# ecmwf-ifs/ectrans

Hardware: AMD Instinct MI355X
Metric: dir+inv transform-pairs/sec, TCo1279 137L x 10 fields; spectral-norm rel-error (higher is better)
Workload: dtype f64

## Files before the change

### ectrans_amd/__init__.py

```python
import ctypes as C
import os

import numpy as np

__all__ = ["TransError", "setup_trans0", "setup_trans", "inv_trans", "dir_trans", "trans_inq", "specnorm",
           "trans_release", "trans_end", "lib", "build", "esetup_trans", "einv_trans", "edir_trans", "etrans_inq"]

_HERE = os.path.dirname(os.path.abspath(__file__))
_LIBPATH = os.path.join(_HERE, "libectrans_mi.so")
_L = None

EMI_MEM_HOST, EMI_MEM_DEVICE, EMI_MEM_AUTO = 0, 1, 2


class TransError(RuntimeError):
    """What the reference would have reported through ABORT_TRANS."""


class _Init(C.Structure):
    _fields_ = [("kmax_resol", C.c_int), ("kprintlev", C.c_int), ("prad", C.c_double), ("nproc", C.c_int),
                ("myproc", C.c_int), ("device", C.c_int), ("nprtrv", C.c_int)]


class _VSets(C.Structure):
    _fields_ = [("kvsetuv", C.POINTER(C.c_int)), ("nuv_g", C.c_int), ("kvsetsc", C.POINTER(C.c_int)), ("nsc_g", C.c_int),
                ("kvsetsc2", C.POINTER(C.c_int)), ("nsc2_g", C.c_int), ("kvsetsc3a", C.POINTER(C.c_int)), ("nsc3a_g", C.c_int),
                ("kvsetsc3b", C.POINTER(C.c_int)), ("nsc3b_g", C.c_int), ("nvar3a_g", C.c_int), ("nvar3b_g", C.c_int)]


class _LegpolIO(C.Structure):
    _fields_ = [("io", C.c_char_p), ("fname", C.c_char_p), ("ptr", C.c_void_p), ("len", C.c_size_t)]


class _Setup(C.Structure):
    _fields_ = [("ksmax", C.c_int), ("kdgl", C.c_int), ("kloen", C.POINTER(C.c_int)), ("kdlon", C.c_int),
                ("precision", C.c_int), ("lduseflt", C.c_int), ("ldll", C.c_int), ("ldstretch", C.c_int),
                ("lduserpnm", C.c_int), ("ldshiftll", C.c_int)]


class _ESetup(C.Structure):
    _fields_ = [("kmsmax", C.c_int), ("ksmax", C.c_int), ("kdgl", C.c_int), ("kloen", C.POINTER(C.c_int)), ("kdlon", C.c_int),
                ("kdgux", C.c_int), ("pexwn", C.c_double), ("peywn", C.c_double), ("precision", C.c_int)]


class _Ext(C.Structure):
    _fields_ = [("sp_dim2", C.c_int), ("gp", C.c_int * 3), ("gpuv", C.c_int * 4), ("gp3a", C.c_int * 4),
                ("gp3b", C.c_int * 4), ("gp2", C.c_int * 3)]


class _Inv(C.Structure):
    _fields_ = [("mem_space", C.c_int), ("spvor", C.c_void_p), ("spdiv", C.c_void_p), ("nf_uv", C.c_int),
                ("spscalar", C.c_void_p), ("nf_scalar", C.c_int), ("spsc3a", C.c_void_p), ("sc3a_nlev", C.c_int),
                ("sc3a_nvar", C.c_int), ("spsc3b", C.c_void_p), ("sc3b_nlev", C.c_int), ("sc3b_nvar", C.c_int),
                ("spsc2", C.c_void_p), ("nf_sc2", C.c_int), ("ldscders", C.c_int), ("ldvorgp", C.c_int),
                ("lddivgp", C.c_int), ("lduvder", C.c_int), ("kproma", C.c_int), ("gp", C.c_void_p),
                ("gp_nfld", C.c_int), ("gpuv", C.c_void_p), ("gp3a", C.c_void_p), ("gp3b", C.c_void_p),
                ("gp2", C.c_void_p), ("stream", C.c_void_p), ("ext", C.POINTER(_Ext)), ("vsets", C.POINTER(_VSets)),
                ("ldlatlon", C.c_int)]


class _Dir(C.Structure):
    _fields_ = [("mem_space", C.c_int), ("spvor", C.c_void_p), ("spdiv", C.c_void_p), ("nf_uv", C.c_int),
                ("spscalar", C.c_void_p), ("nf_scalar", C.c_int), ("spsc3a", C.c_void_p), ("sc3a_nlev", C.c_int),
                ("sc3a_nvar", C.c_int), ("spsc3b", C.c_void_p), ("sc3b_nlev", C.c_int), ("sc3b_nvar", C.c_int),
                ("spsc2", C.c_void_p), ("nf_sc2", C.c_int), ("kproma", C.c_int), ("gp", C.c_void_p),
                ("gp_nfld", C.c_int), ("gpuv", C.c_void_p), ("gp3a", C.c_void_p), ("gp3b", C.c_void_p),
                ("gp2", C.c_void_p), ("stream", C.c_void_p), ("ext", C.POINTER(_Ext)), ("vsets", C.POINTER(_VSets))]


def build(force=False):
    import subprocess
    src = os.path.join(_HERE, "csrc", "ectrans_mi.hip")
    deps = [src] + [os.path.join(_HERE, "csrc", f) for f in ("emi_kernels.h", "emi_kernels_body.h", "emi_mr_body.h", "emi_mr_tables.h", "emi_types.h", "emi_rt.h", "emi_setup.h", "emi_stage.h")]
    deps.append(os.path.join(os.path.dirname(_HERE), "include", "ectrans_mi.h"))
    if not force and os.path.exists(_LIBPATH) and all(os.path.getmtime(_LIBPATH) >= os.path.getmtime(d) for d in deps):
        return _LIBPATH
    hipcc = os.environ.get("HIPCC", "/opt/rocm/bin/hipcc")
    cmd = [hipcc, "--offload-arch=gfx950", "-O3", "-std=c++17", "-fPIC", "-shared", "-o", _LIBPATH, src]
    subprocess.check_call(cmd)
    return _LIBPATH


def source_hash():
    import hashlib
    h = hashlib.sha256()
    files = sorted(os.path.join(_HERE, "csrc", f) for f in os.listdir(os.path.join(_HERE, "csrc")))
    files.append(os.path.join(os.path.dirname(_HERE), "include", "ectrans_mi.h"))
    for f in files:
        if os.path.isfile(f):
            h.update(os.path.basename(f).encode() + b"\0" + open(f, "rb").read())
    return h.hexdigest()[:16]


def _bind(L):
    ip, dp = C.POINTER(C.c_int), C.POINTER(C.c_double)
    L.emi_init.argtypes = [C.POINTER(_Init)]
    L.emi_setup.argtypes = [C.POINTER(_Setup), ip]
    L.emi_setup_legpol.argtypes = [C.POINTER(_Setup), C.POINTER(_LegpolIO), ip]
    L.emi_inq_int.argtypes = [C.c_int, C.c_char_p, ip]
    L.emi_inq_int_array.argtypes = [C.c_int, C.c_char_p, ip, C.c_int]
    L.emi_inq_real_array.argtypes = [C.c_int, C.c_char_p, dp, C.c_int]
    L.emi_inq_legendre.argtypes = [C.c_int, C.c_int, C.c_int, dp, ip, ip]
    L.emi_inv_trans.argtypes = [C.c_int, C.POINTER(_Inv)]
    L.emi_dir_trans.argtypes = [C.c_int, C.POINTER(_Dir)]
    L.emi_specnorm.argtypes = [C.c_int, C.c_int, C.c_void_p, C.c_int, dp]
    L.emi_inv_transad.argtypes = [C.c_int, C.POINTER(_Inv)]
    L.emi_dir_transad.argtypes = [C.c_int, C.POINTER(_Dir)]
    L.emi_release.argtypes = [C.c_int]
    L.emi_finalize.argtypes = []
    L.emi_trim_cache.argtypes = []
    L.emi_last_error.restype = C.c_char_p
    L.emi_work_model.argtypes = [C.c_int, C.c_int, dp, dp, dp]
    L.emi_last_phase_ms.argtypes = [dp]
    L.emi_set_max_batch.argtypes = [C.c_int]
    L.emi_specnorm_partial.argtypes = [C.c_int, C.c_int, C.c_void_p, C.c_int, dp]
    L.emi_gpnorm.argtypes = [C.c_int, C.c_int, C.c_void_p, C.c_int, C.c_int, C.c_int, dp, dp, dp, C.c_int]
    L.emi_vordiv_to_uv.argtypes = [C.c_int, C.c_int, C.c_int, C.c_void_p, C.c_void_p, C.c_void_p, C.c_void_p, C.c_int, C.c_int]
    if hasattr(L, "emi_ptr_space"):
        L.emi_ptr_space.argtypes = [C.c_void_p]
        L.emi_wait.argtypes = [C.c_int]
    L.emi_specnorm_kvset.argtypes = [C.c_int, C.c_int, C.c_void_p, C.c_int, C.POINTER(C.c_int), C.c_int, dp]
    L.emi_set_alltoallv.argtypes = [C.c_void_p, C.c_void_p]
    L.emi_set_profile.argtypes = [C.c_int]
    L.emi_last_phase_launches.argtypes = [ip]
    if hasattr(L, "emi_last_exchange"):
        L.emi_last_exchange.argtypes = [dp, ip, dp]
        L.emi_last_fft_launches.argtypes = [C.POINTER(C.c_longlong)]
    L.emi_crc64.argtypes = [C.c_void_p, C.c_size_t, C.POINTER(C.c_ulonglong)]
    L.emi_set_host_collectives.argtypes = [C.c_void_p, C.c_void_p, C.c_void_p]
    L.emi_dist_spec.argtypes = [C.c_int, C.c_void_p, C.c_int, ip, ip, C.c_void_p]
    L.emi_gath_spec.argtypes = [C.c_int, C.c_void_p, C.c_int, ip, C.c_void_p]
    L.emi_dist_grid.argtypes = [C.c_int, C.c_void_p, C.c_int, ip, ip, C.c_int, C.c_void_p]
    L.emi_gath_grid.argtypes = [C.c_int, C.c_void_p, C.c_int, ip, C.c_int, C.c_void_p]
    L.emi_inq_tasks.argtypes = [ip, ip]
    L.emi_inq_init.argtypes = [ip, dp]
    L.emi_set_nprtrv.argtypes = [C.c_int]
    if hasattr(L, "emi_esetup"):
        L.emi_esetup.argtypes = [C.POINTER(_ESetup), ip]
        L.emi_einv_trans.argtypes = [C.c_int, C.POINTER(_Inv), C.c_void_p, C.c_void_p]
        L.emi_edir_trans.argtypes = [C.c_int, C.POINTER(_Dir), C.c_void_p, C.c_void_p]
    return L


def lib():
    global _L
    if _L is None:
        if not os.path.exists(_LIBPATH):
            raise TransError("libectrans_mi.so is not built (run __graft_entry__.build()); "
                             "ectrans_amd has no CPU implementation")
        _L = _bind(C.CDLL(_LIBPATH))
    return _L


def _use_library_for_tests(path):
    global _L
    _L = _bind(C.CDLL(path))
    return _L


def _chk(rc):
    if rc != 0:
        raise TransError(lib().emi_last_error().decode())


def _is_torch(a):
    return a is not None and type(a).__module__.startswith("torch")


def _ptr(a, space):
    if a is None:
        return None, None
    if _is_torch(a):
        if not a.is_contiguous() or str(a.dtype) != "torch." + space[1]:
            raise TransError("device arrays must be contiguous %s tensors" % space[1])
        if space[0] is None:
            space[0] = EMI_MEM_DEVICE if a.is_cuda else EMI_MEM_HOST
        elif space[0] != (EMI_MEM_DEVICE if a.is_cuda else EMI_MEM_HOST):
            raise TransError("all arrays of one call must live in the same memory space")
        return a.data_ptr(), a
    if not (isinstance(a, np.ndarray) and a.dtype == np.dtype(space[1]) and a.flags.c_contiguous):
        raise TransError("host arrays must be C-contiguous %s numpy arrays" % space[1])
    if space[0] is None:
        space[0] = EMI_MEM_HOST
    elif space[0] != EMI_MEM_HOST:
        raise TransError("all arrays of one call must live in the same memory space")
    return a.ctypes.data, a


def _space(mem_space, space):
    return int(mem_space) if mem_space is not None else space[0] if space[0] is not None else EMI_MEM_HOST


_DIST = {"nproc": 1, "nprtrv": 1, "group": None, "device": None}


def setup_trans0(kmax_resol=1, kprintlev=0, prad=None, device=-1, kprtrw=1, myproc=1, group=None, alltoallv=None,
                 transport="torch", kprtrv=1, **unsupported):
    for k, v in unsupported.items():
        if k.lower() in ("kprgpns", "kprgpew") and v not in (None, 1, kprtrw, kprtrw * kprtrv):
            raise TransError("SETUP_TRANS0: %s=%r: only the W-set decomposition (KPRTRW tasks) is supported" % (k, v))
    nproc_all = kprtrw * max(1, kprtrv)
    if transport == "rccl":
        from . import dist as _dist
        if kprtrv > 1:
            _chk(lib().emi_set_nprtrv(int(kprtrv)))
        _dist.rccl_native_attach(nproc_all, myproc, kmax_resol, kprintlev, prad, device, group)
        _DIST.update(nproc=nproc_all, nprtrv=max(1, kprtrv), group=group if nproc_all > 1 else None,
                     device=("cuda:%d" % device) if nproc_all > 1 and device is not None and device >= 0 else None)
        return
    if nproc_all > 1:
# ... 439 lines not shown
    dt = real_dtype(kresol)
    ns2g, me = trans_inq(kresol, "nspec2g"), trans_inq(kresol, "myproc")
    kto = _roots(kto, kfgathg, "GATH_SPEC:KTO")
    loc = np.ascontiguousarray(_np(pspec), dtype=dt)
    nm = int((kto == me).sum())
    g = np.zeros((nm, ns2g), dtype=dt) if nm else None
    _chk(lib().emi_gath_spec(kresol, None if g is None else g.ctypes.data, kfgathg, _iptr(kto), loc.ctypes.data))
    return None if g is None else np.ascontiguousarray(g.T)


def gath_grid(kresol, pgp, kfgathg, kto=1):
    dt = real_dtype(kresol)
    ngg, me = trans_inq(kresol, "ngptotg"), trans_inq(kresol, "myproc")
    kto = _roots(kto, kfgathg, "GATH_GRID:KTO")
    loc = np.ascontiguousarray(_np(pgp), dtype=dt)
    if loc.ndim != 3 or loc.shape[1] != kfgathg:
        raise TransError("GATH_GRID: PGP must have shape (ngpblks, kfgathg=%d, nproma)" % kfgathg)
    nm = int((kto == me).sum())
    g = np.zeros((nm, ngg), dtype=dt) if nm else None
    _chk(lib().emi_gath_grid(kresol, None if g is None else g.ctypes.data, kfgathg, _iptr(kto), loc.shape[2], loc.ctypes.data))
    return g


def dist_grid(kresol, pgpg, kfdistg, kfrom=1, kproma=None):
    dt = real_dtype(kresol)
    ngl, ngg, me = trans_inq(kresol, "ngptot"), trans_inq(kresol, "ngptotg"), trans_inq(kresol, "myproc")
    kfrom = _roots(kfrom, kfdistg, "DIST_GRID:KFROM")
    mine = np.flatnonzero(kfrom == me)
    g = None
    if mine.size:
        a = _np(pgpg)
        if a.shape[-1] != ngg:
            raise TransError("DIST_GRID: PGPG must have shape (nfld, ngptotg=%d)" % ngg)
        g = np.ascontiguousarray(a[mine], dtype=dt)
    nproma = int(kproma) if kproma else ngl
    out = np.zeros(((ngl - 1) // nproma + 1, kfdistg, nproma), dtype=dt)
    _chk(lib().emi_dist_grid(kresol, None if g is None else g.ctypes.data, kfdistg, _iptr(kfrom), None, nproma, out.ctypes.data))
    return out


def trans_release(kresol):
    _chk(lib().emi_release(kresol))


def trim_cache():
    _chk(lib().emi_trim_cache())


def trans_end():
    _chk(lib().emi_finalize())
    _DIST.update(nproc=1, nprtrv=1, group=None, device=None)


def work_model(kresol, nfields):
    a, b, c = C.c_double(), C.c_double(), C.c_double()
    _chk(lib().emi_work_model(kresol, nfields, C.byref(a), C.byref(b), C.byref(c)))
    return {"legendre_flops": a.value, "fft_flops": b.value, "fourier_bytes": c.value}


def last_phase_ms():
    out = (C.c_double * 3)()
    lib().emi_last_phase_ms(out)
    return list(out)


def last_phase_launches():
    out = (C.c_int * 3)()
    lib().emi_last_phase_launches(out)
    return list(out)


def last_exchange():
    ms, n, b = C.c_double(), C.c_int(), C.c_double()
    lib().emi_last_exchange(C.byref(ms), C.byref(n), C.byref(b))
    return ms.value, n.value, b.value


def last_fft_launches():
    k = C.c_longlong()
    lib().emi_last_fft_launches(C.byref(k))
    return k.value


def set_profile(on):
    lib().emi_set_profile(int(on))


def set_max_batch(n):
    lib().emi_set_max_batch(int(n))
```

### ectrans_amd/csrc/ectrans_mi.hip

```cpp
#include <atomic>
#include <chrono>
#include <cmath>
#include <cstdarg>
#include <cstdio>
#include <map>
#include <memory>
#include <string>
#include <vector>

#include <fcntl.h>
#include <sys/mman.h>
#include <sys/stat.h>
#include <unistd.h>

#include "../../include/ectrans_mi.h"
#include "emi_kernels.h"
#include "emi_setup.h"
#include <dlfcn.h>

struct EmiRoctx {
  int (*push)(const char *) = nullptr;
  int (*pop)() = nullptr;
  bool tried = false;
  void load() {
// ... 131 lines not shown
#ifdef EMI_CPU_EMU
  (void)p;
  return EMI_MEM_HOST;
#else
  if (!p) return EMI_MEM_HOST;
  hipPointerAttribute_t at;
  if (hipPointerGetAttributes(&at, p) != hipSuccess) {
    (void)hipGetLastError();
    return EMI_MEM_HOST;
  }
  return (at.type == hipMemoryTypeDevice || at.type == hipMemoryTypeManaged || at.type == hipMemoryTypeArray) ? EMI_MEM_DEVICE : EMI_MEM_HOST;
#endif
}
static int agree_on_mixed_arrays(const char *who, int ndev, int nhost);
static int resolve_space(const char *who, int mem_space, std::initializer_list<const void *> arrays, int *out, bool collective = false) {
  if (mem_space == EMI_MEM_HOST || mem_space == EMI_MEM_DEVICE) {
    *out = mem_space;
    return 0;
  }
  if (mem_space != EMI_MEM_AUTO) EMI_FAIL(EMI_ERR_ARG, "%s: mem_space = %d (EMI_MEM_HOST, EMI_MEM_DEVICE or EMI_MEM_AUTO)", who, mem_space);
  int ndev = 0, nhost = 0;
  for (const void *q : arrays)
    if (q) (emi_ptr_space(q) == EMI_MEM_DEVICE ? ndev : nhost)++;
  if (collective) {
    if (agree_on_mixed_arrays(who, ndev, nhost)) return EMI_ERR_ARG;
  } else if (ndev && nhost) {
    EMI_FAIL(EMI_ERR_ARG, "%s: %d ARRAYS OF THE CALL ARE IN DEVICE MEMORY AND %d IN HOST MEMORY (all of them must live in one place)", who, ndev, nhost);
  }
  *out = ndev ? EMI_MEM_DEVICE : EMI_MEM_HOST;
  return 0;
}

template <class T>
static int upload(const std::vector<T> &h, T **d) {
  void *p = nullptr;
  if (emi_dev_malloc(&p, h.size() * sizeof(T))) return -1;
  if ((!h.empty() && emi_h2d(p, h.data(), h.size() * sizeof(T), 0)) || emi_stream_sync(0)) {
    emi_dev_free(p);
    return -1;
  }
  *d = (T *)p;
  return 0;
}
struct DevAllocs {
  std::vector<void *> list;
  DevAllocs() = default;
  DevAllocs(const DevAllocs &) = delete;
  DevAllocs &operator=(const DevAllocs &) = delete;
  ~DevAllocs() {
    for (void *p : list) emi_dev_free(p);
  }
  int alloc(void **p, size_t bytes) {
    if (emi_dev_malloc(p, bytes)) return -1;
    list.push_back(*p);
    return 0;
  }
};
template <class T, class F>
static int upload(DevAllocs &owner, const std::vector<T> &h, F *field) {
  T *d = nullptr;
  if (upload(h, &d)) return -1;
  owner.list.push_back(d);
  *field = d;
  return 0;
}

#define EMI_LAUNCH_P(esz, kern, grid, block, lds, st, ...)                     \
  do {                                                                         \
    if ((esz) == 8) {                                                          \
      typedef double RT;                                                       \
      EMI_LAUNCH(emi_f64::kern, grid, block, lds, st, __VA_ARGS__);            \
    } else {                                                                   \
      typedef float RT;                                                        \
      EMI_LAUNCH(emi_f32::kern, grid, block, lds, st, __VA_ARGS__);            \
    }                                                                          \
  } while (0)

struct FftClass {
  int nthr = 0, fbk = 0;
  int hot = 0;
  int r16 = 0;
  int split = 0;
  int mr = 0;
  int gmem = 0;
  long long gm_elems = 0;
  std::vector<int> lats;
  int *d_lats = nullptr;
  FftRowDev *d_rows = nullptr;
  size_t lds = 0;
};
struct LegMaps {
  int2 *d_inv = nullptr, *d_dir = nullptr, *d_inv_wide = nullptr, *d_dir_wide = nullptr;
  long long n_inv = 0, n_dir = 0, n_inv_wide = 0, n_dir_wide = 0;
};

struct Plan {
  Plan() = default;
  Plan(const Plan &) = delete;
  Plan &operator=(const Plan &) = delete;
  ~Plan();
  int nsmax = 0, ndgl = 0, ndgnh = 0;
  bool reduced = false;
  bool ldll = false, shiftll = false;
  bool lam = false;
  int lam_n = 0, kdgux = 0;
  double exwn = 0.0, eywn = 0.0;
  std::vector<int> kntmp;
  std::vector<int> l_kntmp, nesm0;
  LamDev lamdev{};
  int lam_nthr = 0;
  size_t lam_lds = 0;
  double ra = 6371229.0;
  std::vector<int> nloen, nmen, ndglu, procm;
  std::vector<int> latlo;
  std::vector<double> rmu, rw, racthe, cos2;
  int ngptotg = 0, nspec2g = 0;
  int nproc = 1, me = 0;
  int nprv = 1, mev = 0;
  std::vector<int> vlat;
  int vfirst(int w, int v) const { return nprv > 1 ? vlat[(size_t)w * nprv + v] : latlo[w]; }
  int vlast(int w, int v) const { return nprv > 1 ? vlat[(size_t)w * nprv + v + 1] : latlo[w + 1]; }
  long long vpoints(int w, int v) const {
    long long c = 0;
    for (int j = vfirst(w, v); j < vlast(w, v); j++) c += nloen[j];
    return c;
  }
  long long voffset(int v) const {
    long long c = 0;
    for (int j = latlo[me]; j < vfirst(me, v); j++) c += nloen[j];
    return c;
  }
  int nump = 0, nlat = 0, lat0 = 0;
  int ngptot = 0, nspec2 = 0;
  std::vector<int> mval, nasm0;
  std::vector<int> l_nmen, l_gpoff, l_fbase;
  std::vector<int> wbase, wrows, ldp, ldk, lattile_pref, ktile_pref, lbase;
  std::vector<long long> offS, offA, offTS, offTA;
  long long frows = 0, lrows = 0, wrows_total = 0, p_elems = 0, pt_elems = 0;
  std::vector<long long> leg_rows, leg_disp, fft_rows, fft_disp;
  EmiGeomDev g{};
  DevAllocs dev_allocs;
  int esz = 8;
  char *d_P = nullptr, *d_PT = nullptr;
  std::vector<FftPlanDev> fplans;
  std::vector<int> planid;
  FftTabDev ftab{};
  std::vector<FftClass> fclass;
  std::map<int, LegMaps> legmaps;
  char *d_W = nullptr, *d_FBL = nullptr, *d_FBF = nullptr;
  size_t cap_W = 0, cap_FBL = 0, cap_FBF = 0;
  void *d_desc = nullptr;
  size_t cap_desc = 0;
  char *d_fftscr = nullptr;
  size_t cap_fftscr = 0;
#ifndef EMI_CPU_EMU
  hipEvent_t ev_done = nullptr;
#endif
  bool ev_valid = false;
};

Plan::~Plan() {
#ifndef EMI_CPU_EMU
  if (ev_done) (void)hipEventDestroy(ev_done);
#endif
  emi_dev_free(d_W);
  emi_dev_free(d_FBL);
// ... 88 lines not shown
  G.nprtrv = c.nprtrv > 0 ? c.nprtrv : (G.nprtrv_preset > 0 ? G.nprtrv_preset : 1);
  if (G.nproc_all % G.nprtrv != 0)
    EMI_FAIL(EMI_ERR_ARG, "SUMP_TRANS0: NPROC INCONSISTENT WITH NPRTRW (NPROC = %d is not a multiple of NPRTRV = %d)", G.nproc_all, G.nprtrv);
  G.nproc = G.nproc_all / G.nprtrv;
  G.myproc = (G.myproc_all - 1) / G.nprtrv + 1;
  G.mysetv = (G.myproc_all - 1) % G.nprtrv + 1;
#ifndef EMI_CPU_EMU
  int ndev = 0;
  if (hipGetDeviceCount(&ndev) != hipSuccess || ndev == 0)
    EMI_FAIL(EMI_ERR_RUNTIME, "emi_init: no HIP device visible -- libectrans_mi has no CPU path");
  if (c.device >= 0) EMI_CHECK(hipSetDevice(c.device));
#endif
  G.plans.clear();
  G.plans.resize(G.max_resol);
  const char *pe = getenv("EMI_PROFILE");
  G.profile = pe ? atoi(pe) : 0;
  const char *mb = getenv("EMI_MAX_BATCH");
  if (mb) G.max_batch = atoi(mb);
  G.init = true;
  return EMI_SUCCESS;
}


static double mr_radix_ops(int R) {
  switch (R) {
    case 2: return 4; case 3: return 14; case 4: return 16; case 5: return 36; case 7: return 66; case 11: return 150;
    case 13: return 204; case 17: return 336; case 19: return 414; case 23: return 594;
    case 6: return 3 * 4 + 2 * 14 + 12; case 8: return 4 * 4 + 2 * 16 + 18; case 9: return 6 * 14 + 24; case 10: return 5 * 4 + 2 * 36 + 24;
    case 12: return 4 * 14 + 3 * 16 + 36; case 14: return 7 * 4 + 2 * 66 + 36; case 15: return 5 * 14 + 3 * 36 + 48; case 16: return 8 * 16 + 54;
    case 18: return 9 * 4 + 2 * 108 + 48; case 20: return 5 * 16 + 4 * 36 + 72; case 21: return 7 * 14 + 3 * 66 + 72;
    default: return -1;
  }
}
static bool mr_choose(int sz, int esz, int fac[3], int &fbk, int &nthr) {
  std::vector<int> rs = {
#define EMI_MR_ROW(r_) r_,
      EMI_MR_RADICES(EMI_MR_ROW)
  };
#ifdef EMI_MR_RADICES_F32
  if (esz == 4)
    for (int r : {EMI_MR_RADICES_F32(EMI_MR_ROW)}) rs.push_back(r);
#endif
#undef EMI_MR_ROW
  double best = 1e300;
  bool found = false;
  auto consider = [&](int A, int B, int C) {
    const int P1 = (B * C) | 1;
    const size_t per_field = (size_t)A * P1 * 2 * esz;
    if (per_field > 160 * 1024 || A * P1 > 65535) return;
    int fb = 16;
    while (fb > 1 && fb * per_field > 40960) fb >>= 1;
    const int R[3] = {A, B, C};
    for (int nt = 128; nt <= 256; nt += 64) {
      double cost = 0;
      for (int ip = 0; ip < 3; ip++) {
        if (R[ip] == 1) continue;
        const long long nb = (long long)fb * (sz / R[ip]);
        const long long sweeps = (nb + nt - 1) / nt;
        cost += (double)(sweeps * nt) / (double)nb * (mr_radix_ops(R[ip]) / R[ip] + 15.0);
      }
      cost *= 1.0 + 0.5 * (256 - nt) / 64.0;
      if (cost < best * (1.0 - 1e-9) || (cost <= best * (1.0 + 1e-9) && nt > nthr)) {
        best = cost, found = true;
        fac[0] = A, fac[1] = B, fac[2] = C, fbk = fb, nthr = nt;
      }
    }
  };
  for (int A : rs) {
    if (sz % A) continue;
    const int m1 = sz / A;
    if (m1 == 1) consider(A, 1, 1);
    for (int B : rs) {
      if (m1 % B) continue;
      const int C = m1 / B;
      if (C == 1) consider(A, B, 1);
      for (int Cc : rs)
        if (Cc == C) consider(A, B, C);
    }
  }
  return found;
}

struct FftSwitches {
  bool mr, r16, r16s, hot;
  static bool off(const char *name) { return getenv(name) && atoi(getenv(name)) == 0; }
  FftSwitches() : mr(!off("EMI_FFT_MR")), r16(!off("EMI_FFT_R16")), r16s(!off("EMI_FFT_R16S")), hot(!getenv("EMI_FFT_NO_HOT")) {}
};
struct HotPlan {
  int pc, S, nfac, fac[5], nfl;
};
static const HotPlan g_hot_plans[] = {
#define EMI_HOT_ROW(pc_, S_, nf_, a_, b_, c_, d_, e_, nfl_) {pc_, S_, nf_, {a_, b_, c_, d_, e_}, nfl_},
    EMI_HOT_PLAN_LIST(EMI_HOT_ROW)
#undef EMI_HOT_ROW
};
#define EMI_LIST_ROW(r_) r_,
static const int g_r16_list[] = {EMI_R16_LIST(EMI_LIST_ROW)}, g_r16s_list[] = {EMI_R16S_LIST(EMI_LIST_ROW)};
#undef EMI_LIST_ROW

static int fft_fields_40k(size_t per_field) {
  int fbk = 16;
  while (fbk > 1 && fbk * per_field > 40960) fbk >>= 1;
  return fbk;
}
static int fft_threads(size_t lds_bytes) { return lds_bytes <= 40960 ? 256 : (lds_bytes <= 81920 ? 512 : 1024); }

struct FftChoice {
  FftPlanDev pl{};
  int nthr = 0;
  int hot = 0;
  bool gmem = false;
};
static int fft_choose(int n, int esz, const FftSwitches &sw, FftChoice &c) {
  FftPlanDev &pl = c.pl;
  pl.n = n;
  pl.cmode = (n % 2 != 0);
  pl.sz = pl.cmode ? n : n / 2;
  std::vector<int> fac;
  pl.blue = !emi::factorize_smooth(pl.sz, fac);
  pl.S = pl.sz;
  int mr_fbk = 0, mr_nthr = 0, mr_fac[3] = {1, 1, 1};
  if (!pl.cmode && pl.sz >= 2 && sw.mr) pl.mr = mr_choose(pl.sz, esz, mr_fac, mr_fbk, mr_nthr) ? 1 : 0;
  if (pl.mr) {
    pl.blue = 0;
    fac.assign(mr_fac, mr_fac + 3);
  }
  if (!pl.mr && !pl.cmode && sw.r16) {
    const int need = 2 * pl.sz - 1;
    if (need > 1536)
      for (int r : g_r16_list)
        if (!pl.r16 && 256 * r >= need) pl.r16 = r;
    if (!pl.r16 && need > 4096 && pl.sz % 2 == 0 && sw.r16s)
      for (int r : g_r16s_list)
        if (!pl.r16 && 256 * r >= pl.sz - 1) pl.r16 = r, pl.split = 2;
    if (pl.r16) pl.blue = 1;
  }
  if (pl.r16) {
    pl.S = 256 * pl.r16;
    fac.assign(1, pl.r16);
  } else if (pl.blue) {
    pl.S = emi::next_235(2 * pl.sz - 1);
    emi::factorize_smooth(pl.S, fac);
    if (!pl.cmode && sw.hot) {
      long long best = (long long)pl.S * (long long)(fac.size() + 1);
      const HotPlan *pick = nullptr;
      for (const HotPlan &r : g_hot_plans) {
        if (r.S < 2 * pl.sz - 1) continue;
        if (fft_fields_40k((size_t)FFT_LDS_ELEMS(r.S) * 2 * esz) < r.nfl) continue;
        const long long cost = (long long)r.S * (r.nfac + 1);
        if (cost <= best) {
          best = cost;
          pick = &r;
        }
      }
      if (pick) {
        pl.S = pick->S;
        fac.assign(pick->fac, pick->fac + pick->nfac);
      }
    }
  }
  if (pl.S > 65535 || fac.size() > 14) EMI_FAIL(EMI_ERR_UNSUPPORTED, "FFT length %d not supported (work size %d)", n, pl.S);
  pl.nfac = (int)fac.size();
  for (int i = 0; i < pl.nfac; i++) pl.fac[i] = fac[i];
  const size_t per_field = (size_t)FFT_LDS_ELEMS(pl.S) * 2 * esz;
  pl.fbk = fft_fields_40k(per_field);
  c.gmem = pl.fbk * per_field > 160 * 1024 && !pl.mr;
  c.nthr = fft_threads(pl.fbk * per_field);
  if (pl.r16) {
    pl.fbk = 1;
    c.nthr = 16 * pl.r16 > 256 ? roundup(16 * pl.r16, 64) : 256;
  } else if (pl.mr) {
    pl.fbk = mr_fbk;
    c.nthr = mr_nthr;
  } else if (pl.blue && !pl.cmode && !c.gmem && sw.hot) {
    int hot_fbk = 0;
    for (const HotPlan &r : g_hot_plans)
      if (r.S == pl.S && r.nfac == pl.nfac && r.nfl <= pl.fbk && std::equal(r.fac, r.fac + r.nfac, pl.fac)) c.hot = r.pc, hot_fbk = r.nfl;
    if (c.hot) {
      pl.fbk = hot_fbk;
      c.nthr = fft_threads(pl.fbk * per_field);
    }
  }
  for (int i = 0; i < pl.nfac; i++)
    if (!c.hot && !pl.r16 && !pl.mr && (pl.fac[i] == 6 || pl.fac[i] > 8)) EMI_FAIL(EMI_ERR_RUNTIME, "internal: composite FFT radix %d without a specialised kernel (length %d)", pl.fac[i], n);
  return 0;
}

struct FftShared {
  int S, tw_off, perm_off, ptw_off[14];
  std::vector<int> fac;
  int r16 = 0, mr = 0;
};
struct FftTabSizes { size_t tw = 0, ptw = 0, perm = 0, rtw = 0, chirp = 0, bhat = 0; };

static void fft_fill_shared(const FftShared &sh, std::vector<d2> &tw, std::vector<d2> &ptw, std::vector<uint16_t> &perm) {
  const int S = sh.S;
  if (sh.mr) {
    const int A = sh.fac[0], B = sh.fac[1], C = sh.fac[2], P1 = (B * C) | 1;
    auto w = [&](long long e) {
      long double a = 2.0L * (long double)M_PIl * (long double)(e % S) / (long double)S;
      return d2{(double)cosl(a), (double)-sinl(a)};
    };
    d2 *t1 = ptw.data() + sh.ptw_off[0], *t2 = ptw.data() + sh.ptw_off[1];
    for (int k1 = 0; k1 < A; k1++) t1[k1] = w((long long)C * k1);
    for (int q = 0; q < A * B; q++) t2[q] = w((long long)q);
    for (int k = 0; k < S; k++) perm[sh.perm_off + k] = (uint16_t)((k % A) * P1 + ((k / A) % B) * C + k / (A * B));
    return;
  }
  if (sh.r16) {
    d2 *dst = ptw.data() + sh.ptw_off[0];
    for (int row = 0; row < 7; row++) {
      const int mult = row < 3 ? row + 1 : 4 * (row - 2);
      for (int t = 0; t < 256; t++) {
        long double a = 2.0L * (long double)M_PIl * (long double)(((long long)t * mult) % S) / (long double)S;
        *dst++ = d2{(double)cosl(a), (double)-sinl(a)};
      }
    }
    return;
  }
  for (int k = 0; k < S; k++) {
    long double a = 2.0L * (long double)M_PIl * (long double)k / (long double)S;
    tw[sh.tw_off + k] = d2{(double)cosl(a), (double)-sinl(a)};
  }
  long long lenp = 1;
  for (size_t ip = 0; ip < sh.fac.size(); ip++) {
    const int R = sh.fac[ip];
    d2 *dst = ptw.data() + sh.ptw_off[ip];
    if (lenp > 1)
      for (int t = 1; t < R; t++)
        for (long long j = 0; j < lenp; j++) {
          long double a = 2.0L * (long double)M_PIl * (long double)((j * t) % (lenp * R)) / (long double)(lenp * R);
          *dst++ = d2{(double)cosl(a), (double)-sinl(a)};
        }
    lenp *= R;
  }
  std::vector<uint16_t> pm;
  emi::dit_positions(S, sh.fac, pm);
  std::copy(pm.begin(), pm.end(), perm.begin() + sh.perm_off);
}

static void fft_fill_length(const FftPlanDev &pl, const std::vector<uint16_t> &perm, std::vector<d2> &rtw, std::vector<d2> &chirp, std::vector<d2> &bhat) {
  const int n = pl.n;
  const double tpi = 2.0 * M_PI;
  for (int k = 0; k <= pl.sz; k++) {
    double a = tpi * (double)k / (double)n;
    rtw[pl.rtw_off + k] = d2{std::cos(a), -std::sin(a)};
  }
  if (!pl.blue) return;
  d2 *c = chirp.data() + pl.chirp_off;
  const int csz = pl.split ? pl.sz / 2 : pl.sz;
  for (int k = 0; k < csz; k++) {
    long long k2 = ((long long)k * k) % (2LL * csz);
    double a = M_PI * (double)k2 / (double)csz;
    c[k] = d2{std::cos(a), -std::sin(a)};
  }
  const int L = pl.S, r0 = pl.fac[0];
// ... 11 lines not shown
      sr += (long double)c[jj].x * cs;
      si += -(long double)c[jj].y * cs;
    }
    if (pl.r16) {
      const int k0 = k % pl.r16, kk = k / pl.r16, k1 = kk % 16, k2 = kk / 16;
      bh[(size_t)k2 * (16 * pl.r16) + 16 * k0 + k1] = d2{(double)(sr / (long double)L), (double)(si / (long double)L)};
      continue;
    }
    const int p = pm[k];
    bh[(size_t)(p % r0) * (L / r0) + p / r0] = d2{(double)sr, (double)si};
  }
}

static const FftShared &fft_share_tables(const FftPlanDev &pl, std::map<int, int> &sidx, std::vector<FftShared> &shared, FftTabSizes &n) {
  const int skey = pl.S * 16 + (pl.r16 ? 15 : (pl.mr ? 14 : pl.nfac));
  auto si = sidx.find(skey);
  if (si != sidx.end()) return shared[si->second];
  FftShared sh{};
  sh.S = pl.S;
  sh.fac.assign(pl.fac, pl.fac + pl.nfac);
  sh.r16 = pl.r16;
  sh.mr = pl.mr;
  sh.tw_off = (int)n.tw;
  sh.perm_off = (int)n.perm;
  if (pl.mr) {
    const int A = pl.fac[0], B = pl.fac[1];
    sh.ptw_off[0] = (int)n.ptw;
    n.ptw += (size_t)A;
    sh.ptw_off[1] = (int)n.ptw;
    n.ptw += (size_t)A * B;
    sh.ptw_off[2] = (int)n.ptw;
    n.perm += pl.S;
  } else if (pl.r16) {
    sh.ptw_off[0] = (int)n.ptw;
    n.ptw += 7 * 256;
  } else {
    n.tw += pl.S;
    n.perm += pl.S;
    long long lenp = 1;
    for (int ip = 0; ip < pl.nfac; ip++) {
      sh.ptw_off[ip] = (int)n.ptw;
      if (lenp > 1) n.ptw += (size_t)(pl.fac[ip] - 1) * lenp;
      lenp *= pl.fac[ip];
    }
  }
  sidx.emplace(skey, (int)shared.size());
  shared.push_back(sh);
  return shared.back();
}

static int build_fft_plans(Plan &P) {
  const FftSwitches sw;
  std::map<int, int> idx;
  std::map<int, int> sidx;
  std::vector<FftShared> shared;
  FftTabSizes nt;
  P.planid.assign(P.nlat, 0);
  for (int j = 0; j < P.nlat; j++) {
    const int n = P.nloen[P.lat0 + j];
    auto it = idx.find(n);
    if (it != idx.end()) {
      P.planid[j] = it->second;
      continue;
    }
    FftChoice c;
    if (int rc = fft_choose(n, P.esz, sw, c)) return rc;
    FftPlanDev &pl = c.pl;
    const FftShared &sh = fft_share_tables(pl, sidx, shared, nt);
    pl.tw_off = sh.tw_off;
    pl.perm_off = sh.perm_off;
    for (int ip = 0; ip < pl.nfac; ip++) pl.ptw_off[ip] = sh.ptw_off[ip];
    pl.rtw_off = (int)nt.rtw;
    nt.rtw += pl.sz + 1;
    if (pl.blue) {
      pl.chirp_off = (int)nt.chirp;
      nt.chirp += pl.split ? pl.sz / 2 : pl.sz;
      pl.bhat_off = (int)nt.bhat;
      nt.bhat += pl.S;
    }
    if (nt.tw > 0x7fffffffULL || nt.ptw > 0x7fffffffULL || nt.bhat > 0x7fffffffULL) EMI_FAIL(EMI_ERR_UNSUPPORTED, "FFT tables too large");
    int cls = -1;
    for (size_t k = 0; k < P.fclass.size(); k++) {
      const FftClass &fc = P.fclass[k];
      if (fc.nthr == c.nthr && fc.fbk == pl.fbk && fc.hot == c.hot && fc.r16 == pl.r16 && fc.split == pl.split && fc.mr == pl.mr && fc.gmem == (int)c.gmem) cls = (int)k;
    }
    if (cls < 0) {
      cls = (int)P.fclass.size();
      P.fclass.emplace_back();
      FftClass &fc = P.fclass[cls];
      fc.nthr = c.nthr, fc.fbk = pl.fbk, fc.hot = c.hot, fc.r16 = pl.r16, fc.split = pl.split, fc.mr = pl.mr, fc.gmem = c.gmem;
    }
    pl.lds_class = cls;
    idx[n] = P.planid[j] = (int)P.fplans.size();
    P.fplans.push_back(pl);
  }
  if (P.lam) {
    FftPlanDev pl{};
    pl.n = pl.sz = pl.S = P.ndgl;
    pl.cmode = 1;
    std::vector<int> fac;
    pl.blue = !emi::factorize_smooth(pl.sz, fac);
    if (pl.blue) {
      pl.S = emi::next_235(2 * pl.sz - 1);
      emi::factorize_smooth(pl.S, fac);
    }
    const int fs = FFT_LDS_ELEMS(pl.S) + 1, fs_max = 160 * 1024 / (4 * P.esz);
    if (fs > fs_max || pl.S > 65535 || fac.size() > 14)
      EMI_FAIL(EMI_ERR_UNSUPPORTED,
               "ESETUP_TRANS: KDGL = %d NEEDS A WORK ARRAY OF %d COMPLEX NUMBERS PER FIELD (KDGL WHERE IT FACTORISES IN 2, 3, 5, 7, ELSE THE CONVOLUTION LENGTH ABOVE 2 KDGL); THE "
               "Y-DIRECTION KERNELS HOLD TWO FIELDS IN THE 160 KIB OF LDS: AT MOST %d",
               P.ndgl, fs, fs_max);
    pl.nfac = (int)fac.size();
    for (int i = 0; i < pl.nfac; i++) pl.fac[i] = fac[i];
    const size_t per_field = (size_t)fs * 2 * P.esz;
    pl.fbk = std::max(2, std::min(16, (int)(80 * 1024 / per_field) / 2 * 2));
    const FftShared &sh = fft_share_tables(pl, sidx, shared, nt);
    pl.tw_off = sh.tw_off;
    pl.perm_off = sh.perm_off;
    for (int ip = 0; ip < pl.nfac; ip++) pl.ptw_off[ip] = sh.ptw_off[ip];
    pl.rtw_off = (int)nt.rtw;
    nt.rtw += pl.sz + 1;
    if (pl.blue) {
      pl.chirp_off = (int)nt.chirp;
      nt.chirp += pl.sz;
      pl.bhat_off = (int)nt.bhat;
      nt.bhat += pl.S;
    }
    pl.lds_class = -1;
    P.lamdev.yplan = (int)P.fplans.size();
    P.lamdev.fbk = pl.fbk;
    P.lamdev.fs = fs;
    P.lam_lds = (size_t)pl.fbk * per_field;
    P.lam_nthr = std::min(512, fft_threads(P.lam_lds));
    P.fplans.push_back(pl);
  }
  std::vector<d2> tw(nt.tw), rtw(nt.rtw), chirp(nt.chirp), bhat(nt.bhat), ptw(nt.ptw);
  std::vector<uint16_t> perm(nt.perm);
  emi::parallel_for((int)shared.size(), [&](int is) { fft_fill_shared(shared[is], tw, ptw, perm); });
  std::vector<int> order(P.fplans.size());
  for (size_t i = 0; i < order.size(); i++) order[i] = (int)i;
  std::sort(order.begin(), order.end(), [&](int a, int b) { return P.fplans[a].n > P.fplans[b].n; });
  emi::parallel_for((int)order.size(), [&](int io) { fft_fill_length(P.fplans[order[io]], perm, rtw, chirp, bhat); });
  for (int j = 0; j < P.nlat; j++) {
    const FftPlanDev &pl = P.fplans[P.planid[j]];
    FftClass &fc = P.fclass[pl.lds_class];
    fc.lats.push_back(j);
    if (fc.gmem)
      fc.gm_elems = std::max(fc.gm_elems, (long long)pl.fbk * FFT_LDS_ELEMS(pl.S));
    else if (fc.mr)
      fc.lds = std::max(fc.lds, (size_t)pl.fbk * pl.fac[0] * ((pl.fac[1] * pl.fac[2]) | 1) * 2 * P.esz);
    else if (fc.r16)
      fc.lds = (size_t)fc.r16 * 272 * 8 + (size_t)((fc.split ? 128 * fc.r16 : 0) + 240) * 2 * P.esz;
    else
      fc.lds = std::max(fc.lds, (size_t)pl.fbk * FFT_LDS_ELEMS(pl.S) * 2 * P.esz);
  }
  std::vector<d2> tw256(15 * 16);
  for (int k1 = 1; k1 < 16; k1++)
    for (int c = 0; c < 16; c++) {
      long double a = 2.0L * (long double)M_PIl * (long double)(c * k1) / 256.0L;
      tw256[(k1 - 1) * 16 + c] = d2{(double)cosl(a), (double)-sinl(a)};
    }
  auto upload_c = [&](const std::vector<d2> &v, const void **d) {
    if (P.esz == 8) return upload(P.dev_allocs, v, d);
    std::vector<f2> w(v.size());
    for (size_t i = 0; i < v.size(); i++) w[i] = f2{(float)v[i].x, (float)v[i].y};
    return upload(P.dev_allocs, w, d);
  };
  FftTabDev &ft = P.ftab;
  if (upload_c(tw, &ft.tw) || upload_c(ptw, &ft.ptw) || upload_c(rtw, &ft.rtw) || upload_c(chirp, &ft.chirp) || upload_c(bhat, &ft.bhat) || upload_c(tw256, &ft.tw256) ||
      upload(P.dev_allocs, perm, &ft.perm) || upload(P.dev_allocs, P.fplans, &ft.plans) || upload(P.dev_allocs, P.planid, &ft.planid))
    return EMI_ERR_RUNTIME;
  for (FftClass &fc : P.fclass) {
    if (upload(P.dev_allocs, fc.lats, &fc.d_lats)) return EMI_ERR_RUNTIME;
// ... 968 lines not shown
        return EMI_ERR_RUNTIME;
      }
      ok = fwrite(buf.data(), 8, buf.size(), f) == buf.size();
    }
  ok = (fclose(f) == 0) && ok;
  if (!ok) EMI_FAIL(EMI_ERR_RUNTIME, "WRITE_LEGPOL:BYTES_IO_WRITE FAILED (%s)", fname);
  return EMI_SUCCESS;
}

struct HostStage {
  size_t esz;
  explicit HostStage(int e) : esz((size_t)e) {}
  std::vector<void *> dev;
  bool failed = false;
  std::vector<std::pair<void *, std::pair<void *, size_t>>> outs;
  ~HostStage() {
    for (void *p : dev) emi_stage::release(p);
  }
  const void *in(const void *h, size_t elems, bool host, emi_stream_t s) {
    if (!h || !host) return h;
    void *d = emi_stage::acquire(elems * esz);
    if (!d) {
      failed = true;
      return nullptr;
    }
    dev.push_back(d);
    if (emi_h2d(d, h, elems * esz, s)) failed = true;
    return d;
  }
  void *out(void *h, size_t elems, bool host, bool preload = false, emi_stream_t s = 0) {
    if (!h || !host) return h;
    void *d = emi_stage::acquire(elems * esz);
    if (!d) {
      failed = true;
      return nullptr;
    }
    dev.push_back(d);
    if (preload && emi_h2d(d, h, elems * esz, s)) failed = true;
    outs.push_back({d, {h, elems * esz}});
    return d;
  }
  void flush(emi_stream_t s) {
    for (auto &o : outs) emi_d2h(o.second.first, o.first, o.second.second, s);
    emi_stream_sync(s);
  }
};

static int grow(Plan &P, char **p, size_t *cap, size_t need, const char *what, emi_stream_t st) {
  if (need <= *cap) return 0;
  plan_quiesce(P);
  emi_stream_sync(0);
  emi_dev_free(*p);
  *p = nullptr;
  *cap = 0;
  void *q;
  if (emi_dev_malloc(&q, need)) EMI_FAIL(EMI_ERR_RUNTIME, "cannot allocate %.2f GiB %s", need / 1073741824.0, what);
  *p = (char *)q;
  *cap = need;
  emi_dev_memset(q, 0, need, st);
  return 0;
}

static int ensure_work(Plan &P, int bfpad, int nfb, emi_stream_t st) {
  const size_t rowb = (size_t)2 * bfpad * P.esz;
  if (grow(P, &P.d_W, &P.cap_W, (size_t)P.wrows_total * rowb, "packed-spectral work buffer", st)) return -1;
  if (P.nproc == 1) {
    if (grow(P, &P.d_FBL, &P.cap_FBL, (size_t)nfb * (P.frows + 1) * rowb, "Fourier work buffer", st)) return -1;
    P.d_FBF = P.d_FBL;
    P.cap_FBF = P.cap_FBL;
  } else {
    if (grow(P, &P.d_FBL, &P.cap_FBL, (size_t)nfb * (P.lrows + 1) * rowb, "Fourier (Legendre-side) exchange buffer", st)) return -1;
    if (grow(P, &P.d_FBF, &P.cap_FBF, (size_t)nfb * P.frows * rowb, "Fourier (FFT-side) exchange buffer", st)) return -1;
  }
  return 0;
}

struct PhaseTimer {
  static const int MAXIV = 4096;
  int n = 0, ncreated = 0;
  bool on = false;
  int kinds[MAXIV];
  double xbytes = 0;
  long long fft_kernels = 0;
#ifndef EMI_CPU_EMU
  hipEvent_t e0[MAXIV], e1[MAXIV];
  void begin(bool on_, bool keep = false) {
    on = on_;
    if (!keep) n = 0, xbytes = 0, fft_kernels = 0;
  }
  int start(int kind, emi_stream_t s) {
    if (!on || n >= MAXIV) return -1;
    if (n >= ncreated) {
      (void)hipEventCreate(&e0[n]);
      (void)hipEventCreate(&e1[n]);
      ncreated = n + 1;
    }
    kinds[n] = kind;
    (void)hipEventRecord(e0[n], s);
    return n++;
  }
  void stop(int iv, emi_stream_t s) {
    if (iv >= 0) (void)hipEventRecord(e1[iv], s);
  }
  void resolve(double *ms3, int *launches) {
    for (int i = 0; i < 4; i++) ms3[i] = 0, launches[i] = 0;
    if (!on) return;
    for (int i = 0; i < n; i++) {
      (void)hipEventSynchronize(e1[i]);
      float ms = 0;
      (void)hipEventElapsedTime(&ms, e0[i], e1[i]);
      ms3[kinds[i]] += ms;
      launches[kinds[i]]++;
    }
  }
#else
  void begin(bool, bool = false) {}
  int start(int, emi_stream_t) { return -1; }
  void stop(int, emi_stream_t) {}
  void resolve(double *ms3, int *launches) {
    for (int i = 0; i < 4; i++) ms3[i] = 0, launches[i] = 0;
  }
#endif
};
static PhaseTimer g_pt;

static int hook_alltoallv(const void *sb, const std::vector<long long> &psc, void *rb, const std::vector<long long> &prc, int npeers, int stride, int first,
                          emi_stream_t st) {
  const int NA = G.nproc_all;
  std::vector<long long> sc(NA, 0), sd(NA, 0), rc(NA, 0), rd(NA, 0);
  for (int k = 0; k < npeers; k++) sc[first + k * stride] = psc[k], rc[first + k * stride] = prc[k];
  for (int r = 1; r < NA; r++) sd[r] = sd[r - 1] + sc[r - 1], rd[r] = rd[r - 1] + rc[r - 1];
  const int iv = g_pt.start(3, st);
  for (int r = 0; r < NA; r++)
    if (g_pt.on && r != G.myproc_all - 1) g_pt.xbytes += (double)sc[r];
  const int rc_hook = G.a2a(G.a2a_user, sb, sc.data(), sd.data(), rb, rc.data(), rd.data(), NA, (void *)st);
  g_pt.stop(iv, st);
  if (rc_hook != 0) EMI_FAIL(EMI_ERR_RUNTIME, "all-to-all-v hook failed");
  return 0;
}
static int exchange(Plan &P, bool to_fft, int ldf, emi_stream_t st, char *FBl, char *FBf) {
  if (P.nproc == 1) return 0;
  const int NP = P.nproc;
  std::vector<long long> sc(NP), rc(NP);
  const long long rowb = (long long)ldf * P.esz;
  for (int r = 0; r < NP; r++) {
    const long long lr = P.leg_rows[r] * rowb, fr = P.fft_rows[r] * rowb;
    sc[r] = to_fft ? lr : fr;
    rc[r] = to_fft ? fr : lr;
  }
  const void *sb = to_fft ? FBl : FBf;
  void *rb = to_fft ? FBf : FBl;
  return hook_alltoallv(sb, sc, rb, rc, NP, P.nprv, P.mev, st);
}

static int ensure_desc(Plan &P, size_t bytes);
static int upload_desc(Plan &P, const std::vector<char> &hd, emi_stream_t st) {
  if (ensure_desc(P, hd.size())) return EMI_ERR_RUNTIME;
#ifdef EMI_CPU_EMU
  emi_h2d(P.d_desc, hd.data(), hd.size(), st);
  return 0;
#else
  static struct {
    void *h[4] = {nullptr, nullptr, nullptr, nullptr};
    size_t cap[4] = {0, 0, 0, 0};
    hipEvent_t ev[4];
    bool init[4] = {false, false, false, false};
    unsigned next = 0;
  } ring;
  const int k = (int)(ring.next++ & 3u);
  if (ring.init[k]) {
    EMI_CHECK(hipEventSynchronize(ring.ev[k]));
  } else {
    EMI_CHECK(hipEventCreateWithFlags(&ring.ev[k], hipEventDisableTiming));
    ring.init[k] = true;
  }
  if (ring.cap[k] < hd.size()) {
    if (ring.h[k]) (void)hipHostFree(ring.h[k]);
    ring.h[k] = nullptr;
    ring.cap[k] = 0;
    const size_t cap = std::max(hd.size(), (size_t)1 << 16);
    EMI_CHECK(hipHostMalloc(&ring.h[k], cap, hipHostMallocDefault));
    ring.cap[k] = cap;
  }
  memcpy(ring.h[k], hd.data(), hd.size());
  EMI_CHECK(hipMemcpyAsync(P.d_desc, ring.h[k], hd.size(), hipMemcpyHostToDevice, (hipStream_t)st));
  EMI_CHECK(hipEventRecord(ring.ev[k], (hipStream_t)st));
  return 0;
#endif
}

static int ensure_desc(Plan &P, size_t bytes) {
  if (bytes <= P.cap_desc) return 0;
  plan_quiesce(P);
  emi_stream_sync(0);
  emi_dev_free(P.d_desc);
  P.d_desc = nullptr;
  size_t cap = std::max(bytes, (size_t)1 << 16);
  if (emi_dev_malloc(&P.d_desc, cap)) return EMI_ERR_RUNTIME;
  P.cap_desc = cap;
  return 0;
}

static int build_tilemap(Plan &P, const std::vector<int> &pref, int nct, int2 **d_map, long long *nblocks, int which = 0) {
  const int nx = 8;
  int gx = 1;
  while (gx * 2 <= std::min(nct, nx)) gx *= 2;
  const int gy = nx / gx;
  std::vector<std::vector<int2>> per(8);
  for (int ml = 0; ml < P.nump; ml++) {
    const bool wide = P.esz == 4 && P.mval[ml] == 0;
    if ((which == 1 && wide) || (which == 2 && !wide)) continue;
    const int nrt = pref[ml + 1] - pref[ml];
    for (int x = 0; x < nx; x++) {
      const int xc = (x + ml) % gx, xl = (x / gx + ml) % gy;
      const int c0 = (int)((long long)xc * nct / gx), c1 = (int)((long long)(xc + 1) * nct / gx);
      for (int rt = xl; rt < nrt; rt += gy)
        for (int ct = c0; ct < c1; ct++) per[x].push_back(int2{ml, (rt << 16) | ct});
    }
  }
  size_t mx = 0;
  for (auto &v : per) mx = std::max(mx, v.size());
  std::vector<int2> map(mx * 8, int2{-1, 0});
  for (int x = 0; x < 8; x++)
    for (size_t k = 0; k < per[x].size(); k++) map[k * 8 + x] = per[x][k];
  *nblocks = (long long)map.size();
  if (map.empty()) {
    *d_map = nullptr;
    return 0;
  }
  return upload(P.dev_allocs, map, d_map);
}

static int leg_tilemaps(Plan &P, int nct, LegMaps **out) {
  auto it = P.legmaps.find(nct);
  if (it == P.legmaps.end()) {
    LegMaps lm;
    const bool split = P.esz == 4;
    if (build_tilemap(P, P.lattile_pref, nct, &lm.d_inv, &lm.n_inv, split ? 1 : 0) || build_tilemap(P, P.ktile_pref, nct, &lm.d_dir, &lm.n_dir, split ? 1 : 0) ||
        (split && (build_tilemap(P, P.lattile_pref, nct, &lm.d_inv_wide, &lm.n_inv_wide, 2) || build_tilemap(P, P.ktile_pref, nct, &lm.d_dir_wide, &lm.n_dir_wide, 2))))
      return EMI_ERR_RUNTIME;
    it = P.legmaps.emplace(nct, lm).first;
  }
  *out = &it->second;
  return 0;
}

static int pick_batch(Plan &P, int nfields, int depth) {
  size_t fr = 0, tot = 0;
  emi_mem_info(&fr, &tot);
  size_t have = fr + P.cap_W + P.cap_FBL + (P.nproc > 1 ? P.cap_FBF : 0) + emi_stage::idle_bytes();
  const int nfb = depth > 1 ? 2 : 1;
  double per_field = (double)(P.wrows_total + nfb * P.frows + (P.nproc > 1 ? nfb * P.lrows : 0)) * 2.0 * P.esz;
  long long cap = (long long)((double)have * 0.85 / per_field);
  cap = cap / 64 * 64;
  if (cap < 64) cap = 64;
  if (G.max_batch > 0) cap = std::min<long long>(cap, std::max(64, roundup(G.max_batch, 64)));
  long long want = roundup((nfields + depth - 1) / depth, 64);
  return (int)std::min(cap, std::max(64LL, want));
}


static int launch_fft(Plan &P, bool inverse, bool adj, const GridFld *d_flds, int nfld, char *FB, int ldf, int nproma,
                       emi_stream_t st) {
  for (size_t c = 0; c < P.fclass.size(); c++) {
    FftClass &fc = P.fclass[c];
    if (fc.lats.empty() || nfld <= 0) continue;
    const int nchunk = (nfld + fc.fbk - 1) / fc.fbk;
    const long long nblocks = (long long)fc.lats.size() * nchunk;
    FftLaunchDev lc{fc.d_lats, (int)fc.lats.size(), nchunk, nblocks, adj ? 1 : 0, fc.d_rows};
    const int nthr = fc.nthr;
    if (g_pt.on) g_pt.fft_kernels++;
    if (fc.gmem) {
      const size_t needb = (size_t)nblocks * fc.gm_elems * 2 * P.esz;
      if (needb > P.cap_fftscr) {
        plan_quiesce(P);
        emi_stream_sync(0);
        emi_dev_free(P.d_fftscr);
        P.d_fftscr = nullptr;
        P.cap_fftscr = 0;
        void *q = nullptr;
        if (emi_dev_malloc(&q, needb)) EMI_FAIL(EMI_ERR_RUNTIME, "cannot allocate %.2f GiB of FFT scratch for the rows that exceed the LDS", needb / 1073741824.0);
        P.d_fftscr = (char *)q;
        P.cap_fftscr = needb;
      }
      if (inverse) {
        if (P.esz == 8)
          EMI_LAUNCH(emi_f64::k_fft_inv_gm, nblocks, nthr, 0, st, P.g, P.ftab, lc, d_flds, nfld, (const double *)FB, ldf, nproma, (d2 *)P.d_fftscr, fc.gm_elems);
        else
          EMI_LAUNCH(emi_f32::k_fft_inv_gm, nblocks, nthr, 0, st, P.g, P.ftab, lc, d_flds, nfld, (const float *)FB, ldf, nproma, (f2 *)P.d_fftscr, fc.gm_elems);
      } else {
        if (P.esz == 8)
          EMI_LAUNCH(emi_f64::k_fft_dir_gm, nblocks, nthr, 0, st, P.g, P.ftab, lc, d_flds, nfld, (double *)FB, ldf, nproma, (d2 *)P.d_fftscr, fc.gm_elems);
        else
          EMI_LAUNCH(emi_f32::k_fft_dir_gm, nblocks, nthr, 0, st, P.g, P.ftab, lc, d_flds, nfld, (float *)FB, ldf, nproma, (f2 *)P.d_fftscr, fc.gm_elems);
      }
      continue;
    }
    if (fc.mr) {
      if (inverse)
        EMI_LAUNCH_P(P.esz, k_fft_inv_mr, nblocks, nthr, fc.lds, st, P.g, P.ftab, lc, d_flds, nfld, (const RT *)FB, ldf, nproma);
      else
        EMI_LAUNCH_P(P.esz, k_fft_dir_mr, nblocks, nthr, fc.lds, st, P.g, P.ftab, lc, d_flds, nfld, (RT *)FB, ldf, nproma);
      continue;
    }
    if (fc.r16 && fc.split) {
      switch (fc.r16) {
#define EMI_R16P_LAUNCH(r_)                                                                                                                 \
  case r_:                                                                                                                                  \
    if (inverse)                                                                                                                            \
      EMI_LAUNCH_P(P.esz, k_fft_inv_r16p<r_>, nblocks, nthr, fc.lds, st, P.g, P.ftab, lc, d_flds, nfld, (const RT *)FB, ldf, nproma);      \
    else                                                                                                                                    \
      EMI_LAUNCH_P(P.esz, k_fft_dir_r16p<r_>, nblocks, nthr, fc.lds, st, P.g, P.ftab, lc, d_flds, nfld, (RT *)FB, ldf, nproma);            \
    break;
        EMI_R16S_LIST(EMI_R16P_LAUNCH)
#undef EMI_R16P_LAUNCH
        default: EMI_FAIL(EMI_ERR_RUNTIME, "internal: no k_fft_*_r16p kernel for R1 = %d", fc.r16);
      }
      continue;
    }
    if (fc.r16) {
      switch (fc.r16) {
#define EMI_R16_LAUNCH(r_)                                                                                                                  \
  case r_:                                                                                                                                  \
    if (inverse)                                                                                                                            \
      EMI_LAUNCH_P(P.esz, k_fft_inv_r16<r_>, nblocks, nthr, fc.lds, st, P.g, P.ftab, lc, d_flds, nfld, (const RT *)FB, ldf, nproma);       \
    else                                                                                                                                    \
      EMI_LAUNCH_P(P.esz, k_fft_dir_r16<r_>, nblocks, nthr, fc.lds, st, P.g, P.ftab, lc, d_flds, nfld, (RT *)FB, ldf, nproma);             \
    break;
        EMI_R16_LIST(EMI_R16_LAUNCH)
#undef EMI_R16_LAUNCH
        default: EMI_FAIL(EMI_ERR_RUNTIME, "internal: no k_fft_*_r16 kernel for R1 = %d", fc.r16);
      }
      continue;
    }
    switch (fc.hot) {
#define EMI_HOT_LAUNCH(pc_, S_, nf_, a_, b_, c_, d_, e_, nfl_)                                                                                       \
  case pc_:                                                                                                                                    \
    if (inverse)                                                                                                                               \
      EMI_LAUNCH_P(P.esz, k_fft_inv_hot<pc_>, nblocks, nthr, fc.lds, st, P.g, P.ftab, lc, d_flds, nfld, (const RT *)FB, ldf, nproma);         \
    else                                                                                                                                       \
      EMI_LAUNCH_P(P.esz, k_fft_dir_hot<pc_>, nblocks, nthr, fc.lds, st, P.g, P.ftab, lc, d_flds, nfld, (RT *)FB, ldf, nproma);               \
    break;
      EMI_HOT_PLAN_LIST(EMI_HOT_LAUNCH)
#undef EMI_HOT_LAUNCH
      default:
        if (inverse)
          EMI_LAUNCH_P(P.esz, k_fft_inv, nblocks, nthr, fc.lds, st, P.g, P.ftab, lc, d_flds, nfld, (const RT *)FB, ldf, nproma);
        else
          EMI_LAUNCH_P(P.esz, k_fft_dir, nblocks, nthr, fc.lds, st, P.g, P.ftab, lc, d_flds, nfld, (RT *)FB, ldf, nproma);
    }
  }
  return 0;
}

struct Pipeline {
#ifndef EMI_CPU_EMU
  hipStream_t sA = nullptr, sB = nullptr, sX = nullptr;
  std::vector<hipEvent_t> ev;
  hipEvent_t fork = nullptr, joinA = nullptr, joinB = nullptr, joinX = nullptr;
  int init() {
    if (sA) return 0;
    EMI_CHECK(hipStreamCreateWithFlags(&sA, hipStreamNonBlocking));
    EMI_CHECK(hipStreamCreateWithFlags(&sB, hipStreamNonBlocking));
    EMI_CHECK(hipStreamCreateWithFlags(&sX, hipStreamNonBlocking));
    EMI_CHECK(hipEventCreateWithFlags(&fork, hipEventDisableTiming));
    EMI_CHECK(hipEventCreateWithFlags(&joinA, hipEventDisableTiming));
    EMI_CHECK(hipEventCreateWithFlags(&joinB, hipEventDisableTiming));
    EMI_CHECK(hipEventCreateWithFlags(&joinX, hipEventDisableTiming));
    return 0;
  }
  hipEvent_t event(size_t i) {
    while (ev.size() <= i) {
      hipEvent_t e;
      (void)hipEventCreateWithFlags(&e, hipEventDisableTiming);
      ev.push_back(e);
    }
    return ev[i];
  }
  void begin(emi_stream_t user) {
    (void)hipEventRecord(fork, user);
    (void)hipStreamWaitEvent(sA, fork, 0);
    (void)hipStreamWaitEvent(sB, fork, 0);
    (void)hipStreamWaitEvent(sX, fork, 0);
  }
  void end(emi_stream_t user) {
    (void)hipEventRecord(joinA, sA);
    (void)hipEventRecord(joinB, sB);
    (void)hipEventRecord(joinX, sX);
    (void)hipStreamWaitEvent(user, joinA, 0);
    (void)hipStreamWaitEvent(user, joinB, 0);
    (void)hipStreamWaitEvent(user, joinX, 0);
  }
  void signal(size_t i, emi_stream_t s) { (void)hipEventRecord(event(i), s); }
  void wait(size_t i, emi_stream_t s) { (void)hipStreamWaitEvent(s, event(i), 0); }
#else
  void *sA = nullptr, *sB = nullptr, *sX = nullptr;
  int init() { return 0; }
  void begin(emi_stream_t) {}
  void end(emi_stream_t) {}
  void signal(size_t, emi_stream_t) {}
  void wait(size_t, emi_stream_t) {}
#endif
};
static Pipeline g_pipe;

static int pipeline_depth(const Plan &P, int nfields) {
  const int cfg = (test_paths() & 2) ? 4 : 1;
#ifdef EMI_CPU_EMU
  (void)P;
  (void)nfields;
  return 1;
#else
  if (nfields < 256) return 1;
  if (P.nproc > 1) {
    static int dcfg = -1;
    if (dcfg < 0) {
      const char *e = getenv("EMI_PIPELINE_DIST");
      dcfg = e ? atoi(e) : 4;
      if (dcfg < 1) dcfg = 1;
    }
    return dcfg;
  }
  return cfg;
#endif
}

#ifndef EMI_CPU_EMU
static int set_lds_attrs() {
  static bool done = false;
  if (done) return 0;
  EMI_CHECK(hipFuncSetAttribute((const void *)emi_f64::k_leg_dir, hipFuncAttributeMaxDynamicSharedMemorySize, 80 * 1024));
  EMI_CHECK(hipFuncSetAttribute((const void *)emi_f32::k_leg_dir, hipFuncAttributeMaxDynamicSharedMemorySize, 80 * 1024));
#define EMI_HOT_ATTR(pc_, S_, nf_, a_, b_, c_, d_, e_, nfl_)                                                                                  \
  EMI_CHECK(hipFuncSetAttribute((const void *)emi_f64::k_fft_inv_hot<pc_>, hipFuncAttributeMaxDynamicSharedMemorySize, 160 * 1024));  \
  EMI_CHECK(hipFuncSetAttribute((const void *)emi_f64::k_fft_dir_hot<pc_>, hipFuncAttributeMaxDynamicSharedMemorySize, 160 * 1024));  \
  EMI_CHECK(hipFuncSetAttribute((const void *)emi_f32::k_fft_inv_hot<pc_>, hipFuncAttributeMaxDynamicSharedMemorySize, 160 * 1024));  \
  EMI_CHECK(hipFuncSetAttribute((const void *)emi_f32::k_fft_dir_hot<pc_>, hipFuncAttributeMaxDynamicSharedMemorySize, 160 * 1024));
  EMI_HOT_PLAN_LIST(EMI_HOT_ATTR)
#undef EMI_HOT_ATTR
  EMI_CHECK(hipFuncSetAttribute((const void *)emi_f64::k_lam_inv, hipFuncAttributeMaxDynamicSharedMemorySize, 160 * 1024));
  EMI_CHECK(hipFuncSetAttribute((const void *)emi_f64::k_lam_dir, hipFuncAttributeMaxDynamicSharedMemorySize, 160 * 1024));
  EMI_CHECK(hipFuncSetAttribute((const void *)emi_f32::k_lam_inv, hipFuncAttributeMaxDynamicSharedMemorySize, 160 * 1024));
  EMI_CHECK(hipFuncSetAttribute((const void *)emi_f32::k_lam_dir, hipFuncAttributeMaxDynamicSharedMemorySize, 160 * 1024));
  EMI_CHECK(hipFuncSetAttribute((const void *)emi_f64::k_fft_inv, hipFuncAttributeMaxDynamicSharedMemorySize, 160 * 1024));
  EMI_CHECK(hipFuncSetAttribute((const void *)emi_f64::k_fft_dir, hipFuncAttributeMaxDynamicSharedMemorySize, 160 * 1024));
  EMI_CHECK(hipFuncSetAttribute((const void *)emi_f32::k_fft_inv, hipFuncAttributeMaxDynamicSharedMemorySize, 160 * 1024));
  EMI_CHECK(hipFuncSetAttribute((const void *)emi_f32::k_fft_dir, hipFuncAttributeMaxDynamicSharedMemorySize, 160 * 1024));
  EMI_CHECK(hipFuncSetAttribute((const void *)emi_f64::k_fft_inv_mr, hipFuncAttributeMaxDynamicSharedMemorySize, 160 * 1024));
  EMI_CHECK(hipFuncSetAttribute((const void *)emi_f64::k_fft_dir_mr, hipFuncAttributeMaxDynamicSharedMemorySize, 160 * 1024));
  EMI_CHECK(hipFuncSetAttribute((const void *)emi_f32::k_fft_inv_mr, hipFuncAttributeMaxDynamicSharedMemorySize, 160 * 1024));
  EMI_CHECK(hipFuncSetAttribute((const void *)emi_f32::k_fft_dir_mr, hipFuncAttributeMaxDynamicSharedMemorySize, 160 * 1024));
#define EMI_R16_ATTR(r_)                                                                                                                     \
  EMI_CHECK(hipFuncSetAttribute((const void *)emi_f64::k_fft_inv_r16<r_>, hipFuncAttributeMaxDynamicSharedMemorySize, 160 * 1024));  \
  EMI_CHECK(hipFuncSetAttribute((const void *)emi_f64::k_fft_dir_r16<r_>, hipFuncAttributeMaxDynamicSharedMemorySize, 160 * 1024));  \
  EMI_CHECK(hipFuncSetAttribute((const void *)emi_f32::k_fft_inv_r16<r_>, hipFuncAttributeMaxDynamicSharedMemorySize, 160 * 1024));  \
  EMI_CHECK(hipFuncSetAttribute((const void *)emi_f32::k_fft_dir_r16<r_>, hipFuncAttributeMaxDynamicSharedMemorySize, 160 * 1024));
  EMI_R16_LIST(EMI_R16_ATTR)
#undef EMI_R16_ATTR
#define EMI_R16P_ATTR(r_)                                                                                                                    \
  EMI_CHECK(hipFuncSetAttribute((const void *)emi_f64::k_fft_inv_r16p<r_>, hipFuncAttributeMaxDynamicSharedMemorySize, 160 * 1024)); \
  EMI_CHECK(hipFuncSetAttribute((const void *)emi_f64::k_fft_dir_r16p<r_>, hipFuncAttributeMaxDynamicSharedMemorySize, 160 * 1024)); \
  EMI_CHECK(hipFuncSetAttribute((const void *)emi_f32::k_fft_inv_r16p<r_>, hipFuncAttributeMaxDynamicSharedMemorySize, 160 * 1024)); \
  EMI_CHECK(hipFuncSetAttribute((const void *)emi_f32::k_fft_dir_r16p<r_>, hipFuncAttributeMaxDynamicSharedMemorySize, 160 * 1024));
  EMI_R16S_LIST(EMI_R16P_ATTR)
#undef EMI_R16P_ATTR
  done = true;
  return 0;
}
#else
static int set_lds_attrs() { return 0; }
#endif

struct ScalarRef {
  int arr;
  int lev, var;
};

template <class ARGS>
static int enumerate_scalars(const ARGS &a, const char *who, std::vector<ScalarRef> &sc) {
  sc.clear();
  if (a.spscalar) {
    if (a.spsc3a || a.spsc3b || a.spsc2) EMI_FAIL(EMI_ERR_ARG, "%s : PSPSCALAR AND PSPSC3A/PSPSC3B/PSPSC2 BOTH PRESENT", who);
    for (int i = 0; i < a.nf_scalar; i++) sc.push_back({0, i, 0});
  } else {
    if (a.spsc2)
      for (int i = 0; i < a.nf_sc2; i++) sc.push_back({1, i, 0});
    if (a.spsc3a)
      for (int v = 0; v < a.sc3a_nvar; v++)
        for (int l = 0; l < a.sc3a_nlev; l++) sc.push_back({2, l, v});
    if (a.spsc3b)
      for (int v = 0; v < a.sc3b_nvar; v++)
        for (int l = 0; l < a.sc3b_nlev; l++) sc.push_back({3, l, v});
  }
  return 0;
}

template <class ARGS>
static int check_extents(const char *who, const ARGS &a, int nspec2, int nproma, int ngpblks, int nuv, int nvar_uv, int dmul,
                         int *uv_dim3) {
  *uv_dim3 = nvar_uv;
  const emi_extents_t *e = a.ext;
  if (!e) return 0;
  if (e->sp_dim2 > 0 && e->sp_dim2 < nspec2)
    EMI_FAIL(EMI_ERR_ARG, "%s : SECOND DIMENSION OF A SPECTRAL ARRAY TOO SMALL (%d < NSPEC2 = %d)", who, e->sp_dim2, nspec2);
  auto lead = [&](const char *nm, int d1) {
    if (d1 < nproma) {
      emi_set_error("%s:FIRST DIMENSION OF %s TOO SMALL (%d < %d)", who, nm, d1, nproma);
      return -1;
    }
    if (d1 != nproma) {
      emi_set_error("%s: first extent of %s is %d, NPROMA is %d: pass a packed copy at the C-ABI (the Fortran shim does)", who, nm, d1, nproma);
      return -1;
    }
    return 0;
  };
  if (a.gp) {
    if (lead("PGP", e->gp[0])) return EMI_ERR_ARG;
    if (e->gp[1] != a.gp_nfld) EMI_FAIL(EMI_ERR_ARG, "%s: gp_nfld (%d) is not the second extent of PGP (%d)", who, a.gp_nfld, e->gp[1]);
    if (e->gp[2] < ngpblks) EMI_FAIL(EMI_ERR_ARG, "%s:THIRD DIMENSION OF PGP TOO SMALL (%d < %d)", who, e->gp[2], ngpblks);
  }
  if (a.gpuv) {
    if (lead("PGPUV", e->gpuv[0])) return EMI_ERR_ARG;
    if (e->gpuv[1] != a.nf_uv) EMI_FAIL(EMI_ERR_ARG, "%s:SEC. DIMENSION OF PGPUV INCONSISTENT (%d, IF_UV_G = %d)", who, e->gpuv[1], a.nf_uv);
    if (e->gpuv[2] < nvar_uv) EMI_FAIL(EMI_ERR_ARG, "%s:THIRD DIMENSION OF PGPUV TOO SMALL (%d < %d)", who, e->gpuv[2], nvar_uv);
    if (e->gpuv[3] < ngpblks) EMI_FAIL(EMI_ERR_ARG, "%s:FOURTH DIMENSION OF PGPUV TOO SMALL (%d < %d)", who, e->gpuv[3], ngpblks);
    *uv_dim3 = e->gpuv[2];
    (void)nuv;
  }
  if (a.gp2 && a.nf_sc2 > 0) {
    if (lead("PGP2", e->gp2[0])) return EMI_ERR_ARG;
    if (e->gp2[1] != a.nf_sc2 * dmul) EMI_FAIL(EMI_ERR_ARG, "%s:SEC. DIMENSION OF PGP2 INCONSISTENT (%d, IF_SC2_G = %d)", who, e->gp2[1], a.nf_sc2 * dmul);
    if (e->gp2[2] < ngpblks) EMI_FAIL(EMI_ERR_ARG, "%s:THIRD DIMENSION OF PGP2 TOO SMALL (%d < %d)", who, e->gp2[2], ngpblks);
  }
  if (a.gp3a && a.sc3a_nlev * a.sc3a_nvar > 0) {
// ... 227 lines not shown
    SpecSrc s{};
    s.kind = kind;
    switch (r.arr) {
      case 0: s.a = d.spscalar; s.sa = d.nf_scalar; s.ia = r.lev; break;
      case 1: s.a = d.spsc2; s.sa = d.nf_sc2; s.ia = r.lev; break;
      case 2: s.a = (const char *)d.spsc3a + (size_t)r.var * ns2 * d.sc3a_nlev * P.esz; s.sa = d.sc3a_nlev; s.ia = r.lev; break;
      default: s.a = (const char *)d.spsc3b + (size_t)r.var * ns2 * d.sc3b_nlev * P.esz; s.sa = d.sc3b_nlev; s.ia = r.lev; break;
    }
    return s;
  };
  auto uvsrc = [&](int i, int kind) {
    SpecSrc s{};
    s.kind = kind;
    s.a = d.spvor; s.sa = d.nf_uv; s.ia = i;
    s.b = d.spdiv; s.sb = d.nf_uv; s.ib = i;
    if (kind == SPK_COPY + 100) { s.kind = SPK_COPY; s.a = d.spdiv; }
    return s;
  };
  int l0[GF_N] = {};
  if (f.vorgp) { l0[GF_VOR] = (int)lt.size(); for (int i = 0; i < nuv; i++) lt.push_back(uvsrc(i, SPK_COPY)); }
  if (f.divgp) { l0[GF_DIV] = (int)lt.size(); for (int i = 0; i < nuv; i++) lt.push_back(uvsrc(i, SPK_COPY + 100)); }
  l0[GF_U] = (int)lt.size(); for (int i = 0; i < nuv; i++) lt.push_back(uvsrc(i, adj ? SPK_U_AD : SPK_U));
  l0[GF_V] = (int)lt.size(); for (int i = 0; i < nuv; i++) lt.push_back(uvsrc(i, adj ? SPK_V_AD : SPK_V));
  l0[GF_SC] = (int)lt.size(); for (auto &r : f.sc) lt.push_back(sc_src(r, SPK_COPY));
  if (f.scders) { l0[GF_NSD] = (int)lt.size(); for (auto &r : f.sc) lt.push_back(sc_src(r, SPK_NSD)); }
  l0[GF_UEW] = l0[GF_U], l0[GF_VEW] = l0[GF_V], l0[GF_SCEW] = l0[GF_SC];
  for (GridRef &r : gl) r.g.src = l0[r.grp] + r.i;
  const int nlt = (int)lt.size();

  const int depth = pipeline_depth(P, nlt);
  const int bsz = pick_batch(P, nlt, depth);
  const int nbat = (nlt + bsz - 1) / bsz;
  const int tiles_total = (nlt + 63) / 64;
  const int bfpad = 64 * ((tiles_total + nbat - 1) / nbat);
  std::vector<Batch> bats;
  std::vector<char> hdesc;
  for (int ibat = 0, b0 = 0; ibat < nbat; ibat++) {
    const int tiles_b = tiles_total / nbat + (ibat < tiles_total % nbat ? 1 : 0);
    const int nb = std::min(64 * tiles_b, nlt - b0);
    std::vector<GridFld> bg;
    for (const GridRef &r : gl)
      if (r.g.src >= b0 && r.g.src < b0 + nb) {
        bg.push_back(r.g);
        bg.back().src -= b0;
      }
    Batch bt{};
    bt.ldw = 2 * 64 * tiles_b;
    bt.ntiles = (nb + 63) / 64;
    bt.ns = nb, bt.off_s = append_desc(hdesc, lt.data() + b0, nb);
    bt.ng = (int)bg.size(), bt.off_g = append_desc(hdesc, bg.data(), bg.size());
    bats.push_back(bt);
    b0 += nb;
  }
  auto legendre = [&](const Batch &bt, emi_stream_t s, char *FBl, char *) -> int {
    EmiRange rg(EMI_LBL_LTINV);
    const int ldw = bt.ldw, bfpad_b = bt.ldw / 2;
    const SpecSrc *d_bl = (const SpecSrc *)((char *)P.d_desc + bt.off_s);
    if (P.lam) {
      const int nchunk = (bt.ns + P.lamdev.fbk - 1) / P.lamdev.fbk;
      const int ivl = g_pt.start(1, s);
      EMI_LAUNCH_P(P.esz, k_lam_inv, (long long)P.nump * nchunk, P.lam_nthr, P.lam_lds, s, P.g, P.lamdev, P.ftab, d_bl, bt.ns, (const RT *)d.meanu, (const RT *)d.meanv,
                   (RT *)FBl, ldw, nchunk);
      g_pt.stop(ivl, s);
      return 0;
    }
    int iv = g_pt.start(0, s);
    {
      long long nblk = (long long)P.wrows_total * ((bfpad_b + 255) / 256);
      EMI_LAUNCH_P(P.esz, k_prepack_inv, nblk, 256, 0, s, P.g, d_bl, bt.ns, bfpad_b, (RT *)P.d_W, ldw, (long long)P.wrows_total);
    }
    g_pt.stop(iv, s);
    iv = g_pt.start(1, s);
    LegMaps *lmaps = bt.maps;
    if (lmaps->n_inv_wide > 0)
      EMI_LAUNCH(emi_f32::k_leg_inv_wide, lmaps->n_inv_wide, LG_THREADS, LG_LDS_BYTES + 512, s, P.g, (const int2 *)lmaps->d_inv_wide, (const float *)P.d_W, ldw, (float *)FBl, ldw);
    if (lmaps->n_inv > 0)
      EMI_LAUNCH_P(P.esz, k_leg_inv, lmaps->n_inv, LG_THREADS, LG_LDS_BYTES + 512, s, P.g, (const int2 *)lmaps->d_inv, (const RT *)P.d_W, ldw, (RT *)FBl, ldw);
    g_pt.stop(iv, s);
    return 0;
  };
  auto fft = [&](const Batch &bt, emi_stream_t s, char *, char *FBf, auto &&done) -> int {
    EmiRange rgf(EMI_LBL_FTINV);
    const int iv = g_pt.start(2, s);
    if (launch_fft(P, true, adj, (const GridFld *)((char *)P.d_desc + bt.off_g), bt.ng, FBf, bt.ldw, nproma, s)) return EMI_ERR_RUNTIME;
    g_pt.stop(iv, s);
    done();
    return 0;
  };
  return run_batches(P, d.stream, true, depth > 1 && nbat > 1, bfpad, bats, hdesc, legendre, fft);
}

static int dir_pipeline(Plan &P, const Call &d, const Fields &f, const std::vector<GridRef> &gl, int nproma, bool adj) {
  const size_t ns2 = P.nspec2;
  const int nuv = f.nuv, nsc = (int)f.sc.size();
  std::vector<GridFld> gin;
  std::vector<int> num[GF_N];
  for (int grp = 0; grp < GF_N; grp++) num[grp].assign(gf_uv(grp) ? nuv : nsc, -1);
  for (int grp : {GF_U, GF_V, GF_SC, GF_VOR, GF_DIV, GF_UEW, GF_VEW, GF_NSD, GF_SCEW})
    for (const GridRef &r : gl)
      if (r.grp == grp) {
        num[grp][r.i] = (int)gin.size();
        gin.push_back(r.g);
      }
  const int kf_total = (int)gin.size();
  const int natoms = nuv + nsc;
  const int depth = pipeline_depth(P, kf_total);
  const int cap = pick_batch(P, kf_total, depth);
  std::vector<std::vector<int>> batches;
  {
    std::vector<int> cur;
    for (int at = 0; at < natoms; at++) {
      std::vector<int> fl;
      if (at < nuv) {
        fl = {at, nuv + at};
        for (int x : {num[GF_VOR][at], num[GF_DIV][at], num[GF_UEW][at], num[GF_VEW][at]})
          if (x >= 0) fl.push_back(x);
      } else {
        fl = {2 * nuv + (at - nuv)};
        for (int x : {num[GF_NSD][at - nuv], num[GF_SCEW][at - nuv]})
          if (x >= 0) fl.push_back(x);
      }
      if (!cur.empty() && (int)(cur.size() + fl.size()) > cap) {
        batches.push_back(cur);
        cur.clear();
      }
      cur.insert(cur.end(), fl.begin(), fl.end());
    }
    if (!cur.empty()) batches.push_back(cur);
  }
  int maxb = 0;
  for (auto &b : batches) maxb = std::max(maxb, (int)b.size());
  const int bfpad = roundup(maxb, 64);
  const bool fuse_dir = !(test_paths() & 4) && !P.lam;
  std::vector<Batch> bats;
  std::vector<char> hdesc;
  for (auto &b : batches) {
    std::vector<GridFld> bg;
    std::vector<SpecDst> bo;
    std::vector<FuseDst> bf(bfpad, FuseDst{nullptr, 0, 0});
    std::map<int, int> loc;
    for (size_t i = 0; i < b.size(); i++) {
      loc[b[i]] = (int)i;
      bg.push_back(gin[b[i]]);
    }
    auto at_ = [&](int x) { return x >= 0 ? loc[x] : -1; };
    for (size_t i = 0; i < b.size(); i++) {
      int fn = b[i];
      if (fn < nuv) {
        SpecDst v{};
        v.dst = d.spvor; v.stride = d.nf_uv; v.idx = fn; v.kind = adj ? SPO_VOR_AD : SPO_VOR; v.src0 = loc[fn]; v.src1 = loc[nuv + fn];
        v.src2 = at_(num[GF_UEW][fn]); v.src3 = at_(num[GF_VEW][fn]); v.src4 = at_(num[GF_VOR][fn]);
        bo.push_back(v);
        v.dst = d.spdiv; v.kind = adj ? SPO_DIV_AD : SPO_DIV; v.src4 = at_(num[GF_DIV][fn]);
        bo.push_back(v);
      } else if (fn >= 2 * nuv && fn < 2 * nuv + nsc) {
        const int isc = fn - 2 * nuv;
        const ScalarRef &r = f.sc[isc];
        SpecDst sd{};
        sd.kind = SPO_COPY; sd.src0 = (int)i; sd.src1 = sd.src2 = sd.src3 = sd.src4 = -1;
        switch (r.arr) {
          case 0: sd.dst = d.spscalar; sd.stride = d.nf_scalar; sd.idx = r.lev; break;
          case 1: sd.dst = d.spsc2; sd.stride = d.nf_sc2; sd.idx = r.lev; break;
          case 2: sd.dst = (char *)d.spsc3a + (size_t)r.var * ns2 * d.sc3a_nlev * P.esz; sd.stride = d.sc3a_nlev; sd.idx = r.lev; break;
          default: sd.dst = (char *)d.spsc3b + (size_t)r.var * ns2 * d.sc3b_nlev * P.esz; sd.stride = d.sc3b_nlev; sd.idx = r.lev; break;
        }
        if (f.scders) {
          sd.kind = SPO_SC_AD; sd.src1 = at_(num[GF_NSD][isc]); sd.src2 = at_(num[GF_SCEW][isc]);
          bo.push_back(sd);
        } else if (fuse_dir) {
          bf[i] = FuseDst{sd.dst, sd.stride, sd.idx};
        } else {
          bo.push_back(sd);
        }
      }
    }
    Batch bt{};
    bt.ldw = 2 * roundup((int)b.size(), 64);
    bt.ntiles = ((int)b.size() + 63) / 64;
    bt.ng = (int)bg.size(), bt.off_g = append_desc(hdesc, bg.data(), bg.size());
    bt.ns = (int)bo.size(), bt.off_s = append_desc(hdesc, bo.data(), bo.size());
    bt.off_f = append_desc(hdesc, bf.data(), bf.size());
    bats.push_back(bt);
  }
  auto fft = [&](const Batch &bt, emi_stream_t s, char *, char *FBf) -> int {
    EmiRange rg(EMI_LBL_FTDIR);
    const int iv = g_pt.start(2, s);
    if (launch_fft(P, false, adj, (const GridFld *)((char *)P.d_desc + bt.off_g), bt.ng, FBf, bt.ldw, nproma, s)) return EMI_ERR_RUNTIME;
    g_pt.stop(iv, s);
    return 0;
  };
  auto legendre = [&](const Batch &bt, emi_stream_t s, char *FBl, char *, auto &&done) -> int {
    EmiRange rgl(EMI_LBL_LTDIR);
    const int ldw = bt.ldw;
    const long long lrows_call = P.nproc > 1 ? P.lrows : P.frows;
    if (P.lam) {
      const int nchunk = (bt.ng + P.lamdev.fbk - 1) / P.lamdev.fbk;
      const int ivl = g_pt.start(1, s);
      EMI_LAUNCH_P(P.esz, k_lam_dir, (long long)P.nump * nchunk, P.lam_nthr, P.lam_lds, s, P.g, P.lamdev, P.ftab, (const SpecDst *)((char *)P.d_desc + bt.off_s), bt.ns, bt.ng,
                   (RT *)d.meanu, (RT *)d.meanv, (const RT *)FBl, ldw, nchunk);
      g_pt.stop(ivl, s);
      done();
      return 0;
    }
    int iv = g_pt.start(1, s);
    emi_dev_memset(FBl + (size_t)lrows_call * ldw * P.esz, 0, (size_t)ldw * P.esz, s);
    const FuseDst *d_bf = fuse_dir ? (const FuseDst *)((char *)P.d_desc + bt.off_f) : nullptr;
    LegMaps *lmaps = bt.maps;
    if (lmaps->n_dir_wide > 0)
      EMI_LAUNCH(emi_f32::k_leg_dir_wide, lmaps->n_dir_wide, LG_THREADS, leg_dir_lds_bytes(P), s, P.g, (const int2 *)lmaps->d_dir_wide, (const float *)FBl, (int)lrows_call, ldw, (float *)P.d_W, ldw,
                 d_bf);
    if (lmaps->n_dir > 0)
      EMI_LAUNCH_P(P.esz, k_leg_dir, lmaps->n_dir, LG_THREADS, leg_dir_lds_bytes(P), s, P.g, (const int2 *)lmaps->d_dir, (const RT *)FBl, (int)lrows_call, ldw, (RT *)P.d_W, ldw, d_bf);
    g_pt.stop(iv, s);
    done();
    iv = g_pt.start(0, s);
    if (bt.ns > 0) {
      const SpecDst *d_bo = (const SpecDst *)((char *)P.d_desc + bt.off_s);
      long long nblk = ((long long)P.wrows_total + 3) / 4 * ((bt.ns + 63) / 64);
      EMI_LAUNCH_P(P.esz, k_postpack_dir, nblk, 256, 0, s, P.g, d_bo, bt.ns, (const RT *)P.d_W, ldw, (long long)P.wrows_total);
    }
    g_pt.stop(iv, s);
    return 0;
  };
  return run_batches(P, d.stream, false, depth > 1 && batches.size() > 1, bfpad, bats, hdesc, fft, legendre);
}

static int wset_transform(Plan &P, const Call &c, bool inverse, bool adj, const char *who) {
  Fields f;
  if (account(c, who, inverse, nullptr, f)) return EMI_ERR_ARG;
  if (f.if_gp == 0) return EMI_SUCCESS;
  const int nproma = c.kproma > 0 ? c.kproma : P.ngptot;
  const int ngpblks = (P.ngptot - 1) / nproma + 1;
  int uv_dim3 = f.nvar_uv;
  if (check_extents(who, c, P.nspec2, nproma, ngpblks, f.nuv, f.nvar_uv, f.dmul, &uv_dim3)) return EMI_ERR_ARG;
  if (set_lds_attrs()) return EMI_ERR_RUNTIME;
  const emi_stream_t st = c.stream;
  if (plan_begin(P, st)) return EMI_ERR_RUNTIME;
  const bool host = c.mem_space == EMI_MEM_HOST;
  HostStage hs(P.esz);
  const size_t gsz = (size_t)nproma * ngpblks;
  const bool gpad = gsz != (size_t)P.ngptot;
  Call d;
  int rc = stage(P, hs, c, who, inverse, host && f.nuv, f, gsz, gpad, uv_dim3, d);
  if (rc == EMI_SUCCESS && P.lam && f.nuv > 0) {
    const bool hu = host || emi_ptr_space(c.meanu) == EMI_MEM_HOST, hv = host || emi_ptr_space(c.meanv) == EMI_MEM_HOST;
    d.meanu = inverse ? (void *)hs.in(c.meanu, f.nuv, hu, st) : hs.out(c.meanu, f.nuv, hu, true, st);
    d.meanv = inverse ? (void *)hs.in(c.meanv, f.nuv, hv, st) : hs.out(c.meanv, f.nuv, hv, true, st);
    if (hs.failed) rc = EMI_ERR_RUNTIME;
  }
  if (rc == EMI_SUCCESS) {
    std::vector<GridRef> gl;
    grid_fields(f, d, uv_dim3, gl);
    if (P.lam)
      for (GridRef &r : gl) r.g.mode = r.g.mode == GM_ACOS ? GM_PLAIN : (r.g.mode == GM_EWDER_UV ? GM_EWDER : r.g.mode);
    rc = inverse ? inv_pipeline(P, d, f, gl, nproma, adj) : dir_pipeline(P, d, f, gl, nproma, adj);
  }
  if (plan_end(P, st) && rc == EMI_SUCCESS) rc = EMI_ERR_RUNTIME;
  if (rc != EMI_SUCCESS) return rc;
  if (host || !hs.outs.empty()) hs.flush(st);
#ifndef EMI_CPU_EMU
  EMI_CHECK(hipGetLastError());
#endif
  return EMI_SUCCESS;
}

static int specnorm_sumsq(Plan &P, int mem_space, const void *spec, int nfld, double *sumsq) {
  if (resolve_space("SPECNORM", mem_space, {spec}, &mem_space)) return EMI_ERR_ARG;
  HostStage hs(P.esz);
  if (plan_begin(P, (emi_stream_t)0)) return EMI_ERR_RUNTIME;
  const void *d_sp = hs.in(spec, (size_t)P.nspec2 * nfld, mem_space == EMI_MEM_HOST, 0);
// ... 219 lines not shown
      for (int n = m; n <= N; n++) pairm.push_back(ml);
      ipos += 2 * (N - m + 1);
      for (int n = m; n <= N + 2; n++) eps.push_back(std::sqrt((double)(n * n - m * m) / (double)(4 * n * n - 1)));
    }
  }
  for (int n = 1; n <= N + 2; n++) lapin[n + 1] = -(G.ra * G.ra / (double)(n * (n + 1)));
  const int nspec2 = 2 * (int)pairm.size();
  if (nspec2 == 0) return EMI_SUCCESS;
  if (nspec2_ext < nspec2)
    EMI_FAIL(EMI_ERR_ARG, "VORDIV_TO_UV:SECOND DIMENSION OF PSPVOR / PSPDIV / PSPU / PSPV TOO SMALL (%d < %d spectral coefficients at KSMAX = %d)", nspec2_ext, nspec2,
             ksmax);
  if (resolve_space("VORDIV_TO_UV", mem_space, {spvor, spdiv, spu, spv}, &mem_space)) return EMI_ERR_ARG;
  HostStage hs(precision);
  const bool host = mem_space == EMI_MEM_HOST;
  const void *d_vor = hs.in(spvor, (size_t)nspec2 * nfld, host, 0), *d_div = hs.in(spdiv, (size_t)nspec2 * nfld, host, 0);
  void *d_u = hs.out(spu, (size_t)nspec2 * nfld, host), *d_v = hs.out(spv, (size_t)nspec2 * nfld, host);
  int *d_pairm = nullptr, *d_mval = nullptr, *d_nasm0 = nullptr, *d_ebase = nullptr;
  double *d_eps = nullptr, *d_lapin = nullptr;
  int rc = EMI_SUCCESS;
  if (hs.failed || upload(pairm, &d_pairm) || upload(mval, &d_mval) || upload(nasm0, &d_nasm0) || upload(ebase, &d_ebase) || upload(eps, &d_eps) ||
      upload(lapin, &d_lapin)) {
    emi_set_error("VORDIV_TO_UV: no device memory");
    rc = EMI_ERR_RUNTIME;
  } else {
    Vd2uvDev d{d_pairm, d_mval, d_nasm0, d_ebase, d_eps, d_lapin, N, nspec2, nfld, 1.0 / G.ra};
    const long long nthr = (long long)(nspec2 / 2) * nfld;
    EMI_LAUNCH_P(precision, k_vd2uv, (nthr + 255) / 256, 256, 0, (emi_stream_t)0, d, (const RT *)d_vor, (const RT *)d_div, (RT *)d_u, (RT *)d_v);
    hs.flush(0);
    emi_stream_sync(0);
  }
  for (void *q : {(void *)d_pairm, (void *)d_mval, (void *)d_nasm0, (void *)d_ebase, (void *)d_eps, (void *)d_lapin}) emi_dev_free(q);
  return rc;
}

extern "C" int emi_work_model(int kresol, int nfields, double *leg, double *fft, double *fbytes) {
  Plan *Pp = get_plan(kresol);
  if (!Pp) EMI_FAIL(EMI_ERR_STATE, "emi_work_model: unknown resolution %d", kresol);
  if (Pp->lam) EMI_FAIL(EMI_ERR_UNSUPPORTED, "%s: resolution %d is a limited-area handle (ESETUP_TRANS): this routine serves the spherical transforms only", "emi_work_model", kresol);
  Plan &P = *Pp;
  double s = 0.0;
  for (int ml = 0; ml < P.nump; ml++) {
    const int m = P.mval[ml];
    s += 2.0 * std::min(P.ndgnh, P.ndglu[m]) * (double)(P.nsmax - m + 2) * (m == 0 ? 1.0 : 2.0);
  }
  if (leg) *leg = s * nfields;
  double f = 0.0;
  for (int j = P.lat0; j < P.lat0 + P.nlat; j++) f += 2.5 * P.nloen[j] * std::log2((double)std::max(2, P.nloen[j]));
  if (fft) *fft = f * nfields;
  if (fbytes) *fbytes = (double)P.frows * 2.0 * P.esz * nfields;
  return EMI_SUCCESS;
}

extern "C" int emi_last_phase_ms(double *ms3) {
  int l[4];
  double ms[4];
  g_pt.resolve(ms, l);
  for (int i = 0; i < 3; i++) ms3[i] = ms[i];
  return EMI_SUCCESS;
}

extern "C" int emi_last_phase_launches(int *l3) {
  double ms[4];
  int l[4];
  g_pt.resolve(ms, l);
  for (int i = 0; i < 3; i++) l3[i] = l[i];
  return EMI_SUCCESS;
}

extern "C" int emi_last_exchange(double *ms, int *calls, double *bytes_sent) {
  double m4[4];
  int l[4];
  g_pt.resolve(m4, l);
  if (ms) *ms = m4[3];
  if (calls) *calls = l[3];
  if (bytes_sent) *bytes_sent = g_pt.xbytes;
  return EMI_SUCCESS;
}

extern "C" int emi_last_fft_launches(long long *kernels) {
  if (kernels) *kernels = g_pt.fft_kernels;
  return EMI_SUCCESS;
}

extern "C" int emi_set_profile(int on) {
  G.profile = on;
  g_pt.n = 0;
  g_pt.xbytes = 0;
  g_pt.fft_kernels = 0;
  return EMI_SUCCESS;
}

extern "C" int emi_set_max_batch(int max_fields) {
  G.max_batch = max_fields;
  return EMI_SUCCESS;
}

extern "C" int emi_set_host_collectives(emi_bcast_fn bcast, emi_allgatherv_fn allgatherv, void *user) {
  G.hc_bcast = bcast;
  G.hc_gather = allgatherv;
  G.hc_user = user;
  return EMI_SUCCESS;
}
extern "C" int emi_bcast_host(void *buf, long long bytes, int root) {
  if (!G.init) EMI_FAIL(EMI_ERR_STATE, "emi_bcast_host: SETUP_TRANS0 has not been called");
  if (root < 1 || root > G.nproc_all || bytes < 0 || (bytes > 0 && !buf)) EMI_FAIL(EMI_ERR_ARG, "emi_bcast_host: bad arguments");
  if (G.nproc_all == 1 || bytes == 0) return EMI_SUCCESS;
  if (!G.hc_bcast) EMI_FAIL(EMI_ERR_STATE, "emi_bcast_host: several tasks and no host collectives (emi_set_host_collectives)");
  if (G.hc_bcast(G.hc_user, buf, bytes, root - 1)) EMI_FAIL(EMI_ERR_RUNTIME, "emi_bcast_host: broadcast failed");
  return EMI_SUCCESS;
}
extern "C" int emi_inq_init(int *kmax_resol, double *prad) {
  if (!G.init) EMI_FAIL(EMI_ERR_STATE, "emi_inq_init: SETUP_TRANS0 has not been called");
  if (kmax_resol) *kmax_resol = G.max_resol;
  if (prad) *prad = G.ra;
  return EMI_SUCCESS;
}
extern "C" int emi_inq_tasks(int *nproc, int *myproc) {
  if (!G.init) EMI_FAIL(EMI_ERR_STATE, "emi_inq_tasks: SETUP_TRANS0 has not been called");
  if (nproc) *nproc = G.nproc_all;
  if (myproc) *myproc = G.myproc_all;
  return EMI_SUCCESS;
}
namespace {
struct TaskLayout {
  std::vector<long long> iasm0g;
  std::vector<std::vector<int>> ms;
  std::vector<std::vector<long long>> start;
  std::vector<long long> nspec2, gp0, ngp;
};
TaskLayout task_layout(const Plan &P) {
  TaskLayout L;
  const int N = P.nsmax, NP = P.nproc;
  L.iasm0g.assign(N + 2, 0);
  for (int m = 0; m <= N; m++) L.iasm0g[m + 1] = L.iasm0g[m] + 2LL * (N - m + 1);
  L.ms.assign(NP, {});
  L.start.assign(NP, {});
  L.nspec2.assign(NP, 0);
  for (int m = 0; m <= N; m++) {
    const int t = P.procm[m];
    L.ms[t].push_back(m);
    L.start[t].push_back(L.nspec2[t]);
    L.nspec2[t] += 2LL * (N - m + 1);
  }
  std::vector<long long> cum(P.ndgl + 1, 0);
  for (int j = 0; j < P.ndgl; j++) cum[j + 1] = cum[j] + P.nloen[j];
  L.gp0.assign(NP, 0);
  L.ngp.assign(NP, 0);
  for (int t = 0; t < NP; t++) {
    L.gp0[t] = cum[P.latlo[t]];
    L.ngp[t] = cum[P.latlo[t + 1]] - cum[P.latlo[t]];
  }
  return L;
}
int check_tasks(const Plan &P, const int *k, int nfld, const char *who) {
  if (P.nprv > 1) EMI_FAIL(EMI_ERR_UNSUPPORTED, "%s: not available with NPRTRV > 1", who);
  if (nfld < 0 || (nfld > 0 && !k)) EMI_FAIL(EMI_ERR_ARG, "%s: task list missing", who);
  for (int f = 0; f < nfld; f++)
    if (k[f] < 1 || k[f] > P.nproc) EMI_FAIL(EMI_ERR_ARG, "%s: task %d of field %d outside 1..%d", who, k[f], f + 1, P.nproc);
  if (P.nproc > 1 && (!G.hc_bcast || !G.hc_gather))
    EMI_FAIL(EMI_ERR_STATE, "%s: %d tasks but no host collectives registered (emi_set_host_collectives)", who, P.nproc);
  return 0;
}
int slot_of(const int *ksort, int f, int nfld, const char *who, int *slot) {
  *slot = ksort ? ksort[f] - 1 : f;
  if (*slot < 0 || *slot >= nfld) EMI_FAIL(EMI_ERR_ARG, "%s: KSORT(%d) = %d outside 1..%d", who, f + 1, *slot + 1, nfld);
  return 0;
}
}

template <bool SPEC>
static int dist_impl(int kresol, const void *glob, int nfld, const int *kfrom, const int *ksort, int kproma, void *loc, const char *who) {
// ... 422 lines not shown
```

### ectrans_amd/csrc/emi_kernels.h

```cpp
#pragma once
#include "emi_rt.h"

#include "emi_types.h"
#include <type_traits>
#include "emi_mr_tables.h"
#if defined(EMI_MR_STAMP) && !defined(EMI_CPU_EMU)
__device__ unsigned long long emi_mr_stamp[16];
#endif

namespace emi_f64 {
#define EMI_REAL double
#define EMI_REAL2 d2
#define EMI_ACC4 v4d
#define EMI_MFMA emi_mfma_f64
#define EMI_ACC_ROW(l, i) (((l) >> 4) + 4 * (i))
#define EMI_FFT_WAVES 4
#define EMI_MR_EXTRA(X)
#define EMI_LEG_INV_WAVES 2
#define EMI_LEG_DIR_WAVES 2
#define EMI_LEG_WIDE_KERNEL 0
#include "emi_kernels_body.h"
#undef EMI_MR_EXTRA
#undef EMI_REAL
#undef EMI_REAL2
#undef EMI_ACC4
#undef EMI_MFMA
#undef EMI_ACC_ROW
#undef EMI_FFT_WAVES
#undef EMI_LEG_INV_WAVES
#undef EMI_LEG_DIR_WAVES
#undef EMI_LEG_WIDE_KERNEL
}

namespace emi_f32 {
#define EMI_REAL float
#define EMI_REAL2 f2
#define EMI_ACC4 v4f
#define EMI_MFMA emi_mfma_f32
#define EMI_ACC_ROW(l, i) (4 * ((l) >> 4) + (i))
#define EMI_FFT_WAVES 4
#ifdef EMI_MR_RADICES_F32
#define EMI_MR_EXTRA(X) EMI_MR_RADICES_F32(X)
#else
#define EMI_MR_EXTRA(X)
#endif
#define EMI_LEG_INV_WAVES 3
#define EMI_LEG_DIR_WAVES 3
#define EMI_LEG_WIDE_KERNEL 1
#include "emi_kernels_body.h"
#undef EMI_MR_EXTRA
#undef EMI_REAL
#undef EMI_REAL2
#undef EMI_ACC4
#undef EMI_MFMA
#undef EMI_ACC_ROW
#undef EMI_FFT_WAVES
#undef EMI_LEG_INV_WAVES
#undef EMI_LEG_DIR_WAVES
#undef EMI_LEG_WIDE_KERNEL
}
```

### ectrans_amd/csrc/emi_mr_body.h

```cpp

#if defined(EMI_MR_STAMP) && !defined(EMI_LEG_STAMP) && !defined(EMI_CPU_EMU)
#define MR_STAMP_BEGIN()                  \
  unsigned long long st_acc[10] = {0};    \
  unsigned long long st_prev = __builtin_readcyclecounter()
#define MR_STAMP(i_)                                                  \
  do {                                                                \
    const unsigned long long st_now = __builtin_readcyclecounter();   \
    st_acc[i_] += st_now - st_prev;                                   \
    st_prev = st_now;                                                 \
  } while (0)
#define MR_STAMP_END()                                                                \
  do {                                                                                \
    if (EMI_TID == 0) {                                                               \
      for (int i_ = 0; i_ < 10; i_++) atomicAdd(&emi_mr_stamp[i_ < 7 ? i_ : i_ + 1], st_acc[i_]); \
      atomicAdd(&emi_mr_stamp[7], 1ull);                                              \
    }                                                                                 \
  } while (0)
#else
#define MR_STAMP_BEGIN() ((void)0)
#define MR_STAMP(i_) ((void)0)
#define MR_STAMP_END() ((void)0)
#endif

template <int I, int N, class F>
EMI_DEVFN void mr_for(F &&f) {
  if constexpr (I < N) {
    f(std::integral_constant<int, I>{});
    mr_for<I + 1, N>(f);
  }
}

template <int R, int T>
EMI_DEVFN void mr_mulw(real_t &xr, real_t &xi) {
  constexpr int t = ((T % R) + R) % R;
  if constexpr (t == 0) {
  } else if constexpr (4 * t == R) {
    const real_t a = xr;
    xr = xi, xi = -a;
  } else if constexpr (2 * t == R) {
    xr = -xr, xi = -xi;
  } else if constexpr (4 * t == 3 * R) {
    const real_t a = xr;
    xr = -xi, xi = a;
  } else if constexpr (8 * t == R) {
    constexpr real_t h = (real_t)0.70710678118654752440;
    const real_t a = (xr + xi) * h;
    xi = (xi - xr) * h, xr = a;
  } else if constexpr (8 * t == 3 * R) {
    constexpr real_t h = (real_t)0.70710678118654752440;
    const real_t a = (xi - xr) * h;
    xi = -(xr + xi) * h, xr = a;
  } else if constexpr (8 * t == 5 * R) {
    constexpr real_t h = (real_t)0.70710678118654752440;
    const real_t a = -(xr + xi) * h;
    xi = (xr - xi) * h, xr = a;
  } else if constexpr (8 * t == 7 * R) {
    constexpr real_t h = (real_t)0.70710678118654752440;
    const real_t a = (xr - xi) * h;
    xi = (xr + xi) * h, xr = a;
  } else {
    constexpr real_t c = (real_t)mr_cos<R>(t), s = (real_t)mr_sin<R>(t);
    const real_t a = xr * c + xi * s;
    xi = xi * c - xr * s, xr = a;
  }
}

EMI_DEVFN constexpr int mr_split_a(int R) {
  return R == 6 ? 2 : R == 8 ? 2 : R == 9 ? 3 : R == 10 ? 2 : R == 12 ? 3 : R == 14 ? 2 : R == 15 ? 3 : R == 16 ? 4 : R == 18 ? 2 : R == 20 ? 4 : R == 21 ? 3 : 0;
}

template <int R>
struct MrDft {
  template <class Emit>
  static EMI_DEVFN void run(const real_t *xr, const real_t *xi, Emit &&emit) {
    constexpr int SA = mr_split_a(R);
    if constexpr (R == 1) {
      emit(std::integral_constant<int, 0>{}, xr[0], xi[0]);
    } else if constexpr (R == 2) {
      emit(std::integral_constant<int, 0>{}, xr[0] + xr[1], xi[0] + xi[1]);
      emit(std::integral_constant<int, 1>{}, xr[0] - xr[1], xi[0] - xi[1]);
    } else if constexpr (R == 4) {
      const real_t ar = xr[0] + xr[2], ai = xi[0] + xi[2], br = xr[0] - xr[2], bi = xi[0] - xi[2];
      const real_t cr = xr[1] + xr[3], ci = xi[1] + xi[3], dr = xr[1] - xr[3], di = xi[1] - xi[3];
      emit(std::integral_constant<int, 0>{}, ar + cr, ai + ci);
      emit(std::integral_constant<int, 1>{}, br + di, bi - dr);
      emit(std::integral_constant<int, 2>{}, ar - cr, ai - ci);
      emit(std::integral_constant<int, 3>{}, br - di, bi + dr);
    } else if constexpr (SA == 0) {
      constexpr int M = (R - 1) / 2;
      real_t sr[M], si[M], dr[M], di[M];
      real_t y0r = xr[0], y0i = xi[0];
      mr_for<0, M>([&](auto jc) {
        constexpr int j = decltype(jc)::value;
        sr[j] = xr[j + 1] + xr[R - 1 - j], si[j] = xi[j + 1] + xi[R - 1 - j];
        dr[j] = xr[j + 1] - xr[R - 1 - j], di[j] = xi[j + 1] - xi[R - 1 - j];
        y0r += sr[j], y0i += si[j];
      });
      emit(std::integral_constant<int, 0>{}, y0r, y0i);
      mr_for<1, M + 1>([&](auto kc) {
        constexpr int k = decltype(kc)::value;
        real_t ar = xr[0], ai = xi[0], br = 0, bi = 0;
        mr_for<0, M>([&](auto jc) {
          constexpr int j = decltype(jc)::value;
          constexpr int t = ((j + 1) * k) % R;
          constexpr real_t c = (real_t)mr_cos<R>(t), s = (real_t)mr_sin<R>(t);
          ar += c * sr[j], ai += c * si[j];
          if constexpr (j == 0)
            br = s * dr[j], bi = s * di[j];
          else
            br += s * dr[j], bi += s * di[j];
        });
        emit(std::integral_constant<int, k>{}, ar + bi, ai - br);
        emit(std::integral_constant<int, R - k>{}, ar - bi, ai + br);
      });
    } else {
      constexpr int SB = R / SA;
      real_t tr[R], ti[R];
      mr_for<0, SB>([&](auto nbc) {
        constexpr int nb = decltype(nbc)::value;
        real_t ir[SA], ii[SA];
        mr_for<0, SA>([&](auto nac) {
          constexpr int na = decltype(nac)::value;
          ir[na] = xr[na * SB + nb], ii[na] = xi[na * SB + nb];
        });
        MrDft<SA>::run(ir, ii, [&](auto kac, real_t re, real_t im) {
          constexpr int ka = decltype(kac)::value;
          mr_mulw<R, nb * ka>(re, im);
          tr[nb * SA + ka] = re, ti[nb * SA + ka] = im;
        });
      });
      mr_for<0, SA>([&](auto kac) {
        constexpr int ka = decltype(kac)::value;
        real_t ir[SB], ii[SB];
        mr_for<0, SB>([&](auto nbc) {
          constexpr int nb = decltype(nbc)::value;
          ir[nb] = tr[nb * SA + ka], ii[nb] = ti[nb * SA + ka];
        });
        MrDft<SB>::run(ir, ii, [&](auto kbc, real_t re, real_t im) {
          constexpr int kb = decltype(kbc)::value;
          emit(std::integral_constant<int, ka + SA * kb>{}, re, im);
        });
      });
    }
  }
};

EMI_DEVFN unsigned mr_magic(unsigned D) { return D > 1 ? 0xFFFFFFFFu / D + 1u : 0u; }
EMI_DEVFN unsigned mr_div(unsigned j, unsigned m) { return m ? (unsigned)(((unsigned long long)j * m) >> 32) : j; }

struct MrPassArgs {
  int cnt;
  unsigned mcnt, mD;
  int D, SU, SV, ES;
  const real2 *tw;
  int tw_by_u;
};

EMI_DEVFN real_t *mr_row(const GridFld &gf, long long blk0, unsigned rem0, int nproma) {
  return (real_t *)gf.base + (blk0 * gf.nf_arr + gf.fidx) * (long long)nproma + rem0;
}
EMI_DEVFN bool mr_row_flat(const GridFld &gf, long long blk0, unsigned rem0, int nproma, int n) {
  return (rem0 + (unsigned)n <= (unsigned)nproma) && ((((uintptr_t)mr_row(gf, blk0, rem0, nproma)) & (2 * sizeof(real_t) - 1)) == 0);
}

template <int R, int IO>
EMI_DEVFN void mr_pass(real2 *a, int fs, int nfl, const MrPassArgs &pa, const GridFld *flds, long long blk0, unsigned rem0, int nproma) {
  const int ntot = nfl * pa.cnt;
  for (int gi = EMI_TID; gi < ntot; gi += EMI_NTHREADS) {
    const int f = nfl > 1 ? (int)mr_div((unsigned)gi, pa.mcnt) : 0;
    const int j = gi - f * pa.cnt;
    const int u = pa.D > 1 ? (int)mr_div((unsigned)j, pa.mD) : j;
    const int v = j - u * pa.D;
    real2 *p = a + (long long)f * fs + u * pa.SU + v * pa.SV;
    real_t xr[R], xi[R];
    real2 w = mk2(1, 0);
    if (IO != 1 && pa.tw) {
      EMI_GLOBAL_AS const real2 *tw = (EMI_GLOBAL_AS const real2 *)pa.tw + (pa.tw_by_u ? u : j);
      w = mk2(tw->x, tw->y);
    }
    EMI_GLOBAL_AS real2 *row = nullptr;
    if constexpr (IO != 0) row = (EMI_GLOBAL_AS real2 *)mr_row(flds[f], blk0, rem0, nproma) + j;
    if constexpr (IO == 1) {
      mr_for<0, R>([&](auto rc) {
        constexpr int r = decltype(rc)::value;
        xr[r] = row[pa.cnt * r].x, xi[r] = row[pa.cnt * r].y;
      });
    } else {
      mr_for<0, R>([&](auto rc) {
        constexpr int r = decltype(rc)::value;
        const real2 z = p[r * pa.ES];
        xr[r] = z.x, xi[r] = z.y;
      });
    }
    if (IO != 1 && pa.tw) {
      if constexpr (sizeof(real_t) == 4 && (R > 8)) {
        real_t qr[4], qi[4];
        qr[1] = w.x, qi[1] = w.y;
        mr_for<1, R>([&](auto rc) {
          constexpr int r = decltype(rc)::value;
          if constexpr (r == 2) {
            qr[2] = w.x * w.x - w.y * w.y, qi[2] = 2 * w.x * w.y;
          } else if constexpr (r == 3) {
            qr[3] = qr[2] * w.x - qi[2] * w.y, qi[3] = qr[2] * w.y + qi[2] * w.x;
          } else if constexpr (r == 4) {
            qr[0] = qr[2] * qr[2] - qi[2] * qi[2], qi[0] = 2 * qr[2] * qi[2];
            w = mk2(qr[0], qi[0]);
          } else if constexpr (r > 4) {
            const real_t t0 = qr[r & 3] * w.x - qi[r & 3] * w.y;
            qi[r & 3] = qr[r & 3] * w.y + qi[r & 3] * w.x, qr[r & 3] = t0;
          }
          const real_t t1 = xr[r] * qr[r & 3] - xi[r] * qi[r & 3];
          xi[r] = xr[r] * qi[r & 3] + xi[r] * qr[r & 3], xr[r] = t1;
        });
      } else {
        real_t cr = w.x, ci = w.y;
        mr_for<1, R>([&](auto rc) {
          constexpr int r = decltype(rc)::value;
          if constexpr (r > 1) {
            const real_t t0 = cr * w.x - ci * w.y;
            ci = cr * w.y + ci * w.x, cr = t0;
          }
          const real_t t1 = xr[r] * cr - xi[r] * ci;
          xi[r] = xr[r] * ci + xi[r] * cr, xr[r] = t1;
        });
      }
    }
    MrDft<R>::run(xr, xi, [&](auto kc, real_t re, real_t im) {
      constexpr int k = decltype(kc)::value;
      if constexpr (IO == 2)
// ... 202 lines not shown
        }
#pragma unroll
        for (int e = 0; e < 4; e++) {
          const unsigned k = g0 + (unsigned)(e * NT), k2 = (unsigned)sz - k;
          if (k < (unsigned)npair) {
            real2 zk, zk2;
            fin_pair(xa[e], xb[e], k, k2, fa, fb, fsc, cconj(w4[e]), mk2((real_t)1.0, (real_t)0.0), mk2((real_t)1.0, (real_t)0.0), zk, zk2);
            a[k + (pad ? mr_div(k, mbc) * (unsigned)pad : 0u)] = cconj(zk);
            if (k2 != k && k2 < (unsigned)sz) a[k2 + (pad ? mr_div(k2, mbc) * (unsigned)pad : 0u)] = cconj(zk2);
          }
        }
      }
    } else
    for (int g0 = EMI_TID; g0 < ntot; g0 += 4 * NT) {
      real2 xa[4], xb[4], w4[4];
      real_t fa4[4], fb4[4];
      int kk[4], ff[4];
#pragma unroll
      for (int e = 0; e < 4; e++) {
        const int gi = g0 + e * NT;
        if (gi < ntot) {
          const int k = nfl > 1 ? (int)mr_div((unsigned)gi, mnf) : gi, fl = gi - k * nfl, k2 = sz - k;
          const GridFld gf = flds[f0 + fl];
          kk[e] = k, ff[e] = fl;
          xa[e] = (k <= nmen) ? fin_raw(FB, FROW(k), ldf, gf.src) : mk2(0, 0);
          xb[e] = (k2 <= nmen) ? fin_raw(FB, FROW(k2), ldf, gf.src) : mk2(0, 0);
          w4[e] = rtw[k];
          fin_factors(gf.mode, racthe, fa4[e], fb4[e]);
        }
      }
#pragma unroll
      for (int e = 0; e < 4; e++) {
        if (g0 + e * NT < ntot) {
          const int k = kk[e], k2 = sz - k;
          real2 *af = a + (long long)ff[e] * m.fs;
          real2 zk, zk2;
          fin_pair(xa[e], xb[e], (unsigned)k, (unsigned)k2, fa4[e], fb4[e], Lc.adj ? adjw : (real_t)1.0, cconj(w4[e]), mk2((real_t)1.0, (real_t)0.0), mk2((real_t)1.0, (real_t)0.0), zk, zk2);
          af[k + (pad ? (int)mr_div((unsigned)k, mbc) * pad : 0)] = cconj(zk);
          if (k2 != k && k2 < sz) af[k2 + (pad ? (int)mr_div((unsigned)k2, mbc) * pad : 0)] = cconj(zk2);
        }
      }
    }
  }
  EMI_SYNC();
  bool flat = true;
  for (int fl = 0; fl < nfl; fl++) flat = flat && mr_row_flat(flds[f0 + fl], blk0, rem0, nproma, n);
  const int last = m.C > 1 ? 2 : (m.B > 1 ? 1 : 0);
  if (last == 0 && flat)
    mr_pass_any<2>(m.A, a, m.fs, nfl, mr_args(m, 0, tw1, tw2), flds + f0, blk0, rem0, nproma);
  else
    mr_pass_any<0>(m.A, a, m.fs, nfl, mr_args(m, 0, tw1, tw2), flds + f0, blk0, rem0, nproma);
  if (m.B > 1) {
    EMI_SYNC();
    if (last == 1 && flat)
      mr_pass_any<2>(m.B, a, m.fs, nfl, mr_args(m, 1, tw1, tw2), flds + f0, blk0, rem0, nproma);
    else
      mr_pass_any<0>(m.B, a, m.fs, nfl, mr_args(m, 1, tw1, tw2), flds + f0, blk0, rem0, nproma);
  }
  if (m.C > 1) {
    EMI_SYNC();
    if (flat)
      mr_pass_any<2>(m.C, a, m.fs, nfl, mr_args(m, 2, tw1, tw2), flds + f0, blk0, rem0, nproma);
    else
      mr_pass_any<0>(m.C, a, m.fs, nfl, mr_args(m, 2, tw1, tw2), flds + f0, blk0, rem0, nproma);
  }
  if (!flat) {
    EMI_SYNC();
    const unsigned short *perm = T.perm + pl.perm_off;
    for (int fl = 0; fl < nfl; fl++) {
      const GridRow gr = grid_row(flds[f0 + fl], gp0, nproma);
      const real2 *af = a + (long long)fl * m.fs;
      for (int i = EMI_TID; i < sz; i += EMI_NTHREADS) {
        const real2 y = af[perm[i]];
        if (grid_pair_ok(gr, 2u * i)) {
          *(real2 *)grid_ptr(gr, 2u * i) = mk2(y.x, -y.y);
        } else {
          *grid_ptr(gr, 2u * i) = y.x;
          *grid_ptr(gr, 2u * i + 1) = -y.y;
        }
      }
    }
  }
}
```

### ectrans_amd/csrc/emi_rt.h

```cpp
#pragma once
#include <cstddef>
#include <cstdint>
#include <cstdio>
#include <cstdlib>
#include <cstring>
#include <cmath>

#ifndef EMI_CPU_EMU
#include <hip/hip_runtime.h>

#define EMI_KERNEL __global__
#define EMI_KERNEL_LB(T) __global__ __launch_bounds__(T)
#define EMI_KERNEL_FFT(W) __global__ __attribute__((amdgpu_flat_work_group_size(64, 1024), amdgpu_waves_per_eu(W, W)))
#define EMI_KERNEL_MR(W) __global__ __attribute__((amdgpu_flat_work_group_size(64, 256), amdgpu_waves_per_eu(W, W)))
#define EMI_KERNEL_LB2(T, W) __global__ __attribute__((amdgpu_flat_work_group_size(T, T), amdgpu_waves_per_eu(W, W)))
#define EMI_KERNEL_LAM(W) __global__ __attribute__((amdgpu_flat_work_group_size(64, 512), amdgpu_waves_per_eu(W, W)))
#define EMI_DEVFN __device__ __forceinline__
#define EMI_TID ((int)threadIdx.x)
#define EMI_BID ((int)blockIdx.x)
#define EMI_NTHREADS ((int)blockDim.x)
#define EMI_SYNC() __syncthreads()
#define EMI_WAVE_SYNC()                                   \
  do {                                                    \
    __builtin_amdgcn_fence(__ATOMIC_RELEASE, "wavefront"); \
    __builtin_amdgcn_wave_barrier();                      \
    __builtin_amdgcn_fence(__ATOMIC_ACQUIRE, "wavefront"); \
  } while (0)
#define EMI_GLOBAL_AS __attribute__((address_space(1)))
#define EMI_LDS_DECL extern __shared__ __attribute__((aligned(16))) char emi_lds_raw[]
#define EMI_LDS_SYNC() __asm__ volatile("s_waitcnt lgkmcnt(0)\n\ts_barrier" ::: "memory")
#define EMI_WAVE_FENCE() __asm__ volatile("" ::: "memory")
#define EMI_SCHED_FENCE() __builtin_amdgcn_sched_barrier(0)
#define EMI_FP_STRICT() _Pragma("clang fp contract(off)")

struct EmiBuf {
  __amdgpu_buffer_rsrc_t r;
};
typedef int emi_v4i __attribute__((ext_vector_type(4)));
typedef int emi_v2i __attribute__((ext_vector_type(2)));
EMI_DEVFN EmiBuf emi_buf(const void *p, unsigned bytes) {
  EmiBuf b;
  b.r = __builtin_amdgcn_make_buffer_rsrc((void *)p, 0, bytes, 0x00020000);
  return b;
}
EMI_DEVFN EmiBuf emi_buf_all(const void *p) { return emi_buf(p, 0xFFFFFFFCu); }
template <class V>
EMI_DEVFN V emi_buf_ld(const EmiBuf &b, unsigned voff, unsigned soff) {
  static_assert(sizeof(V) == 16 || sizeof(V) == 8, "emi_buf_ld: 8- or 16-byte values");
  if constexpr (sizeof(V) == 16)
    return __builtin_bit_cast(V, __builtin_amdgcn_raw_buffer_load_b128(b.r, voff, soff, 0));
  else
    return __builtin_bit_cast(V, __builtin_amdgcn_raw_buffer_load_b64(b.r, voff, soff, 0));
}
template <class V>
EMI_DEVFN void emi_buf_st(const EmiBuf &b, unsigned voff, unsigned soff, V v) {
  static_assert(sizeof(V) == 16 || sizeof(V) == 8, "emi_buf_st: 8- or 16-byte values");
  if constexpr (sizeof(V) == 16)
    __builtin_amdgcn_raw_buffer_store_b128(__builtin_bit_cast(emi_v4i, v), b.r, voff, soff, 0);
  else
    __builtin_amdgcn_raw_buffer_store_b64(__builtin_bit_cast(emi_v2i, v), b.r, voff, soff, 0);
}
EMI_DEVFN int emi_uniform(int x) { return __builtin_amdgcn_readfirstlane(x); }
EMI_DEVFN const char *emi_uniform_ptr(const void *p) {
  const unsigned long long a = (unsigned long long)p;
  const unsigned lo = __builtin_amdgcn_readfirstlane((unsigned)a), hi = __builtin_amdgcn_readfirstlane((unsigned)(a >> 32));
  return (const char *)(((unsigned long long)hi << 32) | lo);
}
template <class V>
EMI_DEVFN V emi_ld_sv(const char *ubase, unsigned voff) {
  return *(const EMI_GLOBAL_AS V *)((const EMI_GLOBAL_AS char *)ubase + voff);
}
EMI_DEVFN int emi_ld_const(const int *tab, int idx) { return ((const __attribute__((address_space(4))) int *)tab)[idx]; }
#define EMI_PRIO_HI() __builtin_amdgcn_s_setprio(1)
#define EMI_PRIO_LO() __builtin_amdgcn_s_setprio(0)
#define EMI_OPAQUE(x) __asm__ volatile("" : "+v"(x))
#define EMI_LDS_PTR (emi_lds_raw)

typedef double v4d __attribute__((ext_vector_type(4)));
typedef double d2 __attribute__((ext_vector_type(2)));
typedef float v4f __attribute__((ext_vector_type(4)));
typedef float f2 __attribute__((ext_vector_type(2)));

EMI_DEVFN v4d emi_mfma_f64(double a, double b, v4d c) {
  return __builtin_amdgcn_mfma_f64_16x16x4f64(a, b, c, 0, 0, 0);
}
EMI_DEVFN v4f emi_mfma_f32(float a, float b, v4f c) {
  return __builtin_amdgcn_mfma_f32_16x16x4f32(a, b, c, 0, 0, 0);
}

typedef hipStream_t emi_stream_t;

#define EMI_CHECK(expr)                                                                 \
  do {                                                                                  \
    hipError_t e_ = (expr);                                                             \
    if (e_ != hipSuccess) {                                                             \
      emi_set_error("%s failed: %s (%s:%d)", #expr, hipGetErrorString(e_), __FILE__, __LINE__); \
      return -1;                                                                        \
    }                                                                                   \
  } while (0)

#define EMI_LAUNCH(kernel, grid, block, lds, stream, ...) \
  hipLaunchKernelGGL(kernel, dim3((unsigned)(grid)), dim3((unsigned)(block)), (size_t)(lds), (stream), __VA_ARGS__)

#else
#include <omp.h>
#include <vector>

#define EMI_KERNEL
#define EMI_KERNEL_LB(T)
#define EMI_KERNEL_FFT(W)
#define EMI_KERNEL_LB2(T, W)
#define EMI_KERNEL_LAM(W)
#define EMI_KERNEL_MR(W)
#define EMI_DEVFN inline
struct EmuCtx {
  int tid, bid, nthreads;
  char *lds;
  double *sa, *sb;
};
extern thread_local EmuCtx *emu_ctx;
#define EMI_TID (emu_ctx->tid)
#define EMI_BID (emu_ctx->bid)
#define EMI_NTHREADS (emu_ctx->nthreads)
static inline void emu_barrier() {
#pragma omp barrier
}
#define EMI_SYNC() emu_barrier()
#define EMI_WAVE_SYNC() emu_barrier()
#define EMI_LDS_SYNC() emu_barrier()
#define EMI_WAVE_FENCE() emu_barrier()
#define EMI_SCHED_FENCE() ((void)0)
#define EMI_FP_STRICT()
struct EmiBuf {
  const char *p;
  unsigned bytes;
};
inline EmiBuf emi_buf(const void *p, unsigned bytes) { return EmiBuf{(const char *)p, bytes}; }
inline EmiBuf emi_buf_all(const void *p) { return emi_buf(p, 0xFFFFFFFCu); }
template <class V>
inline V emi_buf_ld(const EmiBuf &b, unsigned voff, unsigned soff) {
  V v;
  memset(&v, 0, sizeof(V));
  if ((size_t)voff + sizeof(V) <= b.bytes) memcpy(&v, b.p + voff + soff, sizeof(V));
  return v;
}
template <class V>
inline void emi_buf_st(const EmiBuf &b, unsigned voff, unsigned soff, V v) {
  if ((size_t)voff + sizeof(V) <= b.bytes) memcpy((char *)b.p + voff + soff, &v, sizeof(V));
}
inline int emi_uniform(int x) { return x; }
inline const char *emi_uniform_ptr(const void *p) { return (const char *)p; }
inline int emi_ld_const(const int *tab, int idx) { return tab[idx]; }
template <class V>
inline V emi_ld_sv(const char *ubase, unsigned voff) {
  V v;
  memcpy(&v, ubase + voff, sizeof(V));
  return v;
}
#define EMI_GLOBAL_AS
#define EMI_LDS_DECL
#define EMI_OPAQUE(x) ((void)0)
#define EMI_PRIO_HI() ((void)0)
#define EMI_PRIO_LO() ((void)0)
#define EMI_LDS_PTR (emu_ctx->lds)

typedef double v4d __attribute__((vector_size(32)));
struct __attribute__((aligned(16))) d2 {
  double x, y;
};
struct int2 {
  int x, y;
};
typedef float v4f __attribute__((vector_size(16)));
struct __attribute__((aligned(8))) f2 {
  float x, y;
};

inline v4d emi_mfma_f64(double a, double b, v4d c) {
  EmuCtx *x = emu_ctx;
  int w = x->tid >> 6, l = x->tid & 63;
  x->sa[w * 64 + l] = a;
  x->sb[w * 64 + l] = b;
#pragma omp barrier
  for (int i = 0; i < 4; i++) {
    int row = (l >> 4) + 4 * i, col = l & 15;
    double s = c[i];
    for (int k = 0; k < 4; k++) s += x->sa[w * 64 + k * 16 + row] * x->sb[w * 64 + k * 16 + col];
    c[i] = s;
  }
#pragma omp barrier
  return c;
}
inline v4f emi_mfma_f32(float a, float b, v4f c) {
  EmuCtx *x = emu_ctx;
  int w = x->tid >> 6, l = x->tid & 63;
  x->sa[w * 64 + l] = a;
// ... 48 lines not shown
```

### include/ectrans_mi.h

```cpp
#ifndef ECTRANS_MI_H
#define ECTRANS_MI_H

#include <stddef.h>

#ifdef __cplusplus
extern "C" {
#endif

#define EMI_MEM_HOST 0
#define EMI_MEM_DEVICE 1
#define EMI_MEM_AUTO 2
int emi_ptr_space(const void *p);
int emi_wait(int kresol);

#define EMI_SUCCESS 0
#define EMI_ERR_ARG (-1)
#define EMI_ERR_STATE (-2)
#define EMI_ERR_RUNTIME (-3)
#define EMI_ERR_UNSUPPORTED (-4)

typedef struct {
  int kmax_resol;
  int kprintlev;
  double prad;
// ... 73 lines not shown
  int ldlatlon;
} emi_invtrans_t;
int emi_inv_trans(int kresol, const emi_invtrans_t *args);

typedef struct {
  int mem_space;
  void *spvor, *spdiv;
  int nf_uv;
  void *spscalar;
  int nf_scalar;
  void *spsc3a;
  int sc3a_nlev, sc3a_nvar;
  void *spsc3b;
  int sc3b_nlev, sc3b_nvar;
  void *spsc2;
  int nf_sc2;
  int kproma;
  const void *gp;
  int gp_nfld;
  const void *gpuv;
  const void *gp3a, *gp3b, *gp2;
  void *stream;
  const emi_extents_t *ext;
  const emi_vsets_t *vsets;
} emi_dirtrans_t;
int emi_dir_trans(int kresol, const emi_dirtrans_t *args);

int emi_inv_transad(int kresol, const emi_invtrans_t *args);
int emi_dir_transad(int kresol, const emi_dirtrans_t *args);

typedef struct {
  int kmsmax, ksmax;
  int kdgl;
  const int *kloen;
  int kdlon;
  int kdgux;
  double pexwn, peywn;
  int precision;
} emi_esetup_t;
int emi_esetup(const emi_esetup_t *cfg, int *kresol);
int emi_einv_trans(int kresol, const emi_invtrans_t *args, const void *meanu, const void *meanv);
int emi_edir_trans(int kresol, const emi_dirtrans_t *args, void *meanu, void *meanv);

int emi_specnorm(int kresol, int mem_space, const void *spec, int nfld, double *norms );

int emi_specnorm_kvset(int kresol, int mem_space, const void *spec, int nfld, const int *kvset, int nfld_g, double *norms_g);
int emi_inq_vsets(int *nprtrw, int *nprtrv, int *mysetw, int *mysetv);

typedef int (*emi_alltoallv_fn)(void *user, const void *sendbuf, const long long *sendcounts, const long long *sdispls,
                                void *recvbuf, const long long *recvcounts, const long long *rdispls, int nproc, void *stream);
int emi_set_alltoallv(emi_alltoallv_fn fn, void *user);
int emi_specnorm_partial(int kresol, int mem_space, const void *spec, int nfld, double *sumsq );

typedef int (*emi_bcast_fn)(void *user, void *buf, long long bytes, int root );
typedef int (*emi_allgatherv_fn)(void *user, const void *sendbuf, long long sendbytes, void *recvbuf, const long long *recvbytes,
                                 const long long *displs, int nproc);
int emi_set_host_collectives(emi_bcast_fn bcast, emi_allgatherv_fn allgatherv, void *user);
int emi_dist_spec(int kresol, const void *specg, int nfld, const int *kfrom, const int *ksort, void *spec);
int emi_gath_spec(int kresol, void *specg, int nfld, const int *kto, const void *spec);
int emi_dist_grid(int kresol, const void *gpg, int nfld, const int *kfrom, const int *ksort, int kproma, void *gp);
int emi_gath_grid(int kresol, void *gpg, int nfld, const int *kto, int kproma, const void *gp);
int emi_inq_tasks(int *nproc, int *myproc);
int emi_inq_init(int *kmax_resol, double *prad);

int emi_release(int kresol);
int emi_finalize(void);
int emi_trim_cache(void);

const char *emi_last_error(void);

int emi_gpnorm(int kresol, int mem_space, const void *gp, int gp_nfld, int kfields, int kproma, double *ave, double *pmin, double *pmax,
               int ave_only);

int emi_vordiv_to_uv(int ksmax, int precision, int mem_space, const void *spvor, const void *spdiv, void *spu, void *spv, int nfld, int nspec2);

int emi_bcast_host(void *buf, long long bytes, int root);

int emi_work_model(int kresol, int nfields, double *legendre_flops_per_direction,
                   double *fft_flops_per_direction, double *fourier_bytes_per_direction);
int emi_last_phase_ms(double *ms3);
int emi_last_phase_launches(int *l3);
int emi_last_exchange(double *ms, int *calls, double *bytes_sent);
int emi_last_fft_launches(long long *kernels);
int emi_set_profile(int on);
int emi_roctx_active(void);
int emi_set_max_batch(int max_fields);

int emi_crc64(const void *data, size_t bytes, unsigned long long *crc);

#ifdef __cplusplus
}
#endif
#endif
```

Before: 3.011.

## Add specialized compile-time mixed-radix FFT kernels for large TCo1279 row lengths

Adds k_fft_inv_mrs/k_fft_dir_mrs kernels whose radix factors, thread count and row length are fixed at compile time per plan from a table covering the longest f64 latitude rows. The first direct pass reads the grid row straight from global memory, the last inverse pass writes it straight back, and the direct path prefetches the real-to-complex twiddles so it can use LDS-only barriers. This is meant to cut generic index math, LDS round trips and barrier cost in the dominant FFT rows. The kernels are chosen at runtime only when alignment and offset checks pass, which adds more kernel code and a switch over plan ids.

```diff
diff --git a/ectrans_amd/__init__.py b/ectrans_amd/__init__.py
--- a/ectrans_amd/__init__.py
+++ b/ectrans_amd/__init__.py
@@ -71,7 +71,7 @@
 def build(force=False):
     import subprocess
     src = os.path.join(_HERE, "csrc", "ectrans_mi.hip")
-    deps = [src] + [os.path.join(_HERE, "csrc", f) for f in ("emi_kernels.h", "emi_kernels_body.h", "emi_mr_body.h", "emi_mr_tables.h", "emi_types.h", "emi_rt.h", "emi_setup.h", "emi_stage.h")]
+    deps = [src] + [os.path.join(_HERE, "csrc", f) for f in ("emi_kernels.h", "emi_kernels_body.h", "emi_mr_body.h", "emi_mr_tables.h", "emi_mrs_list.h", "emi_types.h", "emi_rt.h", "emi_setup.h", "emi_stage.h")]
     deps.append(os.path.join(os.path.dirname(_HERE), "include", "ectrans_mi.h"))
     if not force and os.path.exists(_LIBPATH) and all(os.path.getmtime(_LIBPATH) >= os.path.getmtime(d) for d in deps):
         return _LIBPATH
@@ -126,6 +126,8 @@
     if hasattr(L, "emi_last_exchange"):
         L.emi_last_exchange.argtypes = [dp, ip, dp]
         L.emi_last_fft_launches.argtypes = [C.POINTER(C.c_longlong)]
+    if hasattr(L, "emi_last_fft_mrs_launches"):
+        L.emi_last_fft_mrs_launches.argtypes = [C.POINTER(C.c_longlong)]
     L.emi_crc64.argtypes = [C.c_void_p, C.c_size_t, C.POINTER(C.c_ulonglong)]
     L.emi_set_host_collectives.argtypes = [C.c_void_p, C.c_void_p, C.c_void_p]
     L.emi_dist_spec.argtypes = [C.c_int, C.c_void_p, C.c_int, ip, ip, C.c_void_p]
@@ -731,6 +733,12 @@
     return k.value
 
 
+def last_fft_mrs_launches():
+    k = C.c_longlong()
+    lib().emi_last_fft_mrs_launches(C.byref(k))
+    return k.value
+
+
 def set_profile(on):
     lib().emi_set_profile(int(on))
 
diff --git a/ectrans_amd/csrc/ectrans_mi.hip b/ectrans_amd/csrc/ectrans_mi.hip
--- a/ectrans_amd/csrc/ectrans_mi.hip
+++ b/ectrans_amd/csrc/ectrans_mi.hip
@@ -237,6 +237,7 @@
   int r16 = 0;
   int split = 0;
   int mr = 0;
+  int mrs = 0;
   int gmem = 0;
   long long gm_elems = 0;
   std::vector<int> lats;
@@ -491,10 +492,17 @@
 }
 
 struct FftSwitches {
-  bool mr, r16, r16s, hot;
+  bool mr, mrs, r16, r16s, hot;
   static bool off(const char *name) { return getenv(name) && atoi(getenv(name)) == 0; }
-  FftSwitches() : mr(!off("EMI_FFT_MR")), r16(!off("EMI_FFT_R16")), r16s(!off("EMI_FFT_R16S")), hot(!getenv("EMI_FFT_NO_HOT")) {}
+  FftSwitches() : mr(!off("EMI_FFT_MR")), mrs(!off("EMI_FFT_MRS")), r16(!off("EMI_FFT_R16")), r16s(!off("EMI_FFT_R16S")), hot(!getenv("EMI_FFT_NO_HOT")) {}
 };
+struct MrsPlanRow {
+  int n, fac[3], nthr, fbk;
+};
+#define EMI_MRS_ROW(id_, n_, a_, b_, c_, nt_, fbk_) {n_, {a_, b_, c_}, nt_, fbk_},
+static const MrsPlanRow g_mrs_plans_f64[] = {EMI_MRS_PLAN_LIST_F64(EMI_MRS_ROW){0, {0, 0, 0}, 0, 0}};
+static const MrsPlanRow g_mrs_plans_f32[] = {EMI_MRS_PLAN_LIST_F32(EMI_MRS_ROW){0, {0, 0, 0}, 0, 0}};
+#undef EMI_MRS_ROW
 struct HotPlan {
   int pc, S, nfac, fac[5], nfl;
 };
@@ -518,6 +526,7 @@
   FftPlanDev pl{};
   int nthr = 0;
   int hot = 0;
+  int mrs = 0;
   bool gmem = false;
 };
 static int fft_choose(int n, int esz, const FftSwitches &sw, FftChoice &c) {
@@ -581,6 +590,9 @@
   } else if (pl.mr) {
     pl.fbk = mr_fbk;
     c.nthr = mr_nthr;
+    if (sw.mrs)
+      for (const MrsPlanRow *r = esz == 8 ? g_mrs_plans_f64 : g_mrs_plans_f32; r->n; r++)
+        if (r->n == n && std::equal(r->fac, r->fac + 3, mr_fac) && r->nthr == mr_nthr && r->fbk == mr_fbk) c.mrs = 1;
   } else if (pl.blue && !pl.cmode && !c.gmem && sw.hot) {
     int hot_fbk = 0;
     for (const HotPlan &r : g_hot_plans)
@@ -758,13 +770,13 @@
     int cls = -1;
     for (size_t k = 0; k < P.fclass.size(); k++) {
       const FftClass &fc = P.fclass[k];
-      if (fc.nthr == c.nthr && fc.fbk == pl.fbk && fc.hot == c.hot && fc.r16 == pl.r16 && fc.split == pl.split && fc.mr == pl.mr && fc.gmem == (int)c.gmem) cls = (int)k;
+      if (fc.nthr == c.nthr && fc.fbk == pl.fbk && fc.hot == c.hot && fc.r16 == pl.r16 && fc.split == pl.split && fc.mr == pl.mr && fc.mrs == c.mrs && fc.gmem == (int)c.gmem) cls = (int)k;
     }
     if (cls < 0) {
       cls = (int)P.fclass.size();
       P.fclass.emplace_back();
       FftClass &fc = P.fclass[cls];
-      fc.nthr = c.nthr, fc.fbk = pl.fbk, fc.hot = c.hot, fc.r16 = pl.r16, fc.split = pl.split, fc.mr = pl.mr, fc.gmem = c.gmem;
+      fc.nthr = c.nthr, fc.fbk = pl.fbk, fc.hot = c.hot, fc.r16 = pl.r16, fc.split = pl.split, fc.mr = pl.mr, fc.mrs = c.mrs, fc.gmem = c.gmem;
     }
     pl.lds_class = cls;
     idx[n] = P.planid[j] = (int)P.fplans.size();
@@ -1899,11 +1911,12 @@
   int kinds[MAXIV];
   double xbytes = 0;
   long long fft_kernels = 0;
+  long long mrs_kernels = 0;
 #ifndef EMI_CPU_EMU
   hipEvent_t e0[MAXIV], e1[MAXIV];
   void begin(bool on_, bool keep = false) {
     on = on_;
-    if (!keep) n = 0, xbytes = 0, fft_kernels = 0;
+    if (!keep) n = 0, xbytes = 0, fft_kernels = 0, mrs_kernels = 0;
   }
   int start(int kind, emi_stream_t s) {
     if (!on || n >= MAXIV) return -1;
@@ -1931,7 +1944,10 @@
     }
   }
 #else
-  void begin(bool, bool = false) {}
+  void begin(bool on_, bool keep = false) {
+    on = on_;
+    if (!keep) xbytes = 0, fft_kernels = 0, mrs_kernels = 0;
+  }
   int start(int, emi_stream_t) { return -1; }
   void stop(int, emi_stream_t) {}
   void resolve(double *ms3, int *launches) {
@@ -2077,7 +2093,19 @@
 }
 
 
-static int launch_fft(Plan &P, bool inverse, bool adj, const GridFld *d_flds, int nfld, char *FB, int ldf, int nproma,
+static bool mrs_call_ok(const Plan &P, const FftClass &fc, const GridFld *h_flds, int nfld, int ldf, int nproma) {
+  if (P.g.fftrow || nproma <= 0 || (nproma & 1)) return false;
+  if ((unsigned long long)(P.nsmax + 2) * (unsigned long long)ldf * P.esz >= 0x7fffffffULL) return false;
+  for (int j : fc.lats) {
+    const long long gp0 = P.l_gpoff[j], rem0 = gp0 % nproma;
+    if (gp0 > 0x7fffffffLL || (rem0 & 1) || rem0 + P.fplans[P.planid[j]].n > nproma) return false;
+  }
+  for (int f = 0; f < nfld; f++)
+    if (((uintptr_t)h_flds[f].base) & (uintptr_t)(2 * P.esz - 1)) return false;
+  return true;
+}
+
+static int launch_fft(Plan &P, bool inverse, bool adj, const GridFld *d_flds, const GridFld *h_flds, int nfld, char *FB, int ldf, int nproma,
                        emi_stream_t st) {
   for (size_t c = 0; c < P.fclass.size(); c++) {
     FftClass &fc = P.fclass[c];
@@ -2113,6 +2141,14 @@
       }
       continue;
     }
+    if (fc.mr && fc.mrs && mrs_call_ok(P, fc, h_flds, nfld, ldf, nproma)) {
+      if (g_pt.on) g_pt.mrs_kernels++;
+      if (inverse)
+        EMI_LAUNCH_P(P.esz, k_fft_inv_mrs, nblocks, nthr, fc.lds, st, P.ftab, lc, d_flds, (const RT *)FB, ldf, nproma);
+      else
+        EMI_LAUNCH_P(P.esz, k_fft_dir_mrs, nblocks, nthr, fc.lds, st, P.ftab, lc, d_flds, (RT *)FB, ldf, nproma);
+      continue;
+    }
     if (fc.mr) {
       if (inverse)
         EMI_LAUNCH_P(P.esz, k_fft_inv_mr, nblocks, nthr, fc.lds, st, P.g, P.ftab, lc, d_flds, nfld, (const RT *)FB, ldf, nproma);
@@ -2267,6 +2303,10 @@
   EMI_CHECK(hipFuncSetAttribute((const void *)emi_f64::k_fft_dir_mr, hipFuncAttributeMaxDynamicSharedMemorySize, 160 * 1024));
   EMI_CHECK(hipFuncSetAttribute((const void *)emi_f32::k_fft_inv_mr, hipFuncAttributeMaxDynamicSharedMemorySize, 160 * 1024));
   EMI_CHECK(hipFuncSetAttribute((const void *)emi_f32::k_fft_dir_mr, hipFuncAttributeMaxDynamicSharedMemorySize, 160 * 1024));
+  EMI_CHECK(hipFuncSetAttribute((const void *)emi_f64::k_fft_inv_mrs, hipFuncAttributeMaxDynamicSharedMemorySize, 160 * 1024));
+  EMI_CHECK(hipFuncSetAttribute((const void *)emi_f64::k_fft_dir_mrs, hipFuncAttributeMaxDynamicSharedMemorySize, 160 * 1024));
+  EMI_CHECK(hipFuncSetAttribute((const void *)emi_f32::k_fft_inv_mrs, hipFuncAttributeMaxDynamicSharedMemorySize, 160 * 1024));
+  EMI_CHECK(hipFuncSetAttribute((const void *)emi_f32::k_fft_dir_mrs, hipFuncAttributeMaxDynamicSharedMemorySize, 160 * 1024));
 #define EMI_R16_ATTR(r_)                                                                                                                     \
   EMI_CHECK(hipFuncSetAttribute((const void *)emi_f64::k_fft_inv_r16<r_>, hipFuncAttributeMaxDynamicSharedMemorySize, 160 * 1024));  \
   EMI_CHECK(hipFuncSetAttribute((const void *)emi_f64::k_fft_dir_r16<r_>, hipFuncAttributeMaxDynamicSharedMemorySize, 160 * 1024));  \
@@ -2660,7 +2700,7 @@
   auto fft = [&](const Batch &bt, emi_stream_t s, char *, char *FBf, auto &&done) -> int {
     EmiRange rgf(EMI_LBL_FTINV);
     const int iv = g_pt.start(2, s);
-    if (launch_fft(P, true, adj, (const GridFld *)((char *)P.d_desc + bt.off_g), bt.ng, FBf, bt.ldw, nproma, s)) return EMI_ERR_RUNTIME;
+    if (launch_fft(P, true, adj, (const GridFld *)((char *)P.d_desc + bt.off_g), (const GridFld *)(hdesc.data() + bt.off_g), bt.ng, FBf, bt.ldw, nproma, s)) return EMI_ERR_RUNTIME;
     g_pt.stop(iv, s);
     done();
     return 0;
@@ -2763,7 +2803,7 @@
   auto fft = [&](const Batch &bt, emi_stream_t s, char *, char *FBf) -> int {
     EmiRange rg(EMI_LBL_FTDIR);
     const int iv = g_pt.start(2, s);
-    if (launch_fft(P, false, adj, (const GridFld *)((char *)P.d_desc + bt.off_g), bt.ng, FBf, bt.ldw, nproma, s)) return EMI_ERR_RUNTIME;
+    if (launch_fft(P, false, adj, (const GridFld *)((char *)P.d_desc + bt.off_g), (const GridFld *)(hdesc.data() + bt.off_g), bt.ng, FBf, bt.ldw, nproma, s)) return EMI_ERR_RUNTIME;
     g_pt.stop(iv, s);
     return 0;
   };
@@ -3149,11 +3189,17 @@
   return EMI_SUCCESS;
 }
 
+extern "C" int emi_last_fft_mrs_launches(long long *kernels) {
+  if (kernels) *kernels = g_pt.mrs_kernels;
+  return EMI_SUCCESS;
+}
+
 extern "C" int emi_set_profile(int on) {
   G.profile = on;
   g_pt.n = 0;
   g_pt.xbytes = 0;
   g_pt.fft_kernels = 0;
+  g_pt.mrs_kernels = 0;
   return EMI_SUCCESS;
 }
 
diff --git a/ectrans_amd/csrc/emi_kernels.h b/ectrans_amd/csrc/emi_kernels.h
--- a/ectrans_amd/csrc/emi_kernels.h
+++ b/ectrans_amd/csrc/emi_kernels.h
@@ -4,6 +4,7 @@
 #include "emi_types.h"
 #include <type_traits>
 #include "emi_mr_tables.h"
+#include "emi_mrs_list.h"
 #if defined(EMI_MR_STAMP) && !defined(EMI_CPU_EMU)
 __device__ unsigned long long emi_mr_stamp[16];
 #endif
@@ -16,11 +17,13 @@
 #define EMI_ACC_ROW(l, i) (((l) >> 4) + 4 * (i))
 #define EMI_FFT_WAVES 4
 #define EMI_MR_EXTRA(X)
+#define EMI_MRS_PLAN_LIST(X) EMI_MRS_PLAN_LIST_F64(X)
 #define EMI_LEG_INV_WAVES 2
 #define EMI_LEG_DIR_WAVES 2
 #define EMI_LEG_WIDE_KERNEL 0
 #include "emi_kernels_body.h"
 #undef EMI_MR_EXTRA
+#undef EMI_MRS_PLAN_LIST
 #undef EMI_REAL
 #undef EMI_REAL2
 #undef EMI_ACC4
@@ -44,11 +47,13 @@
 #else
 #define EMI_MR_EXTRA(X)
 #endif
+#define EMI_MRS_PLAN_LIST(X) EMI_MRS_PLAN_LIST_F32(X)
 #define EMI_LEG_INV_WAVES 3
 #define EMI_LEG_DIR_WAVES 3
 #define EMI_LEG_WIDE_KERNEL 1
 #include "emi_kernels_body.h"
 #undef EMI_MR_EXTRA
+#undef EMI_MRS_PLAN_LIST
 #undef EMI_REAL
 #undef EMI_REAL2
 #undef EMI_ACC4
diff --git a/ectrans_amd/csrc/emi_mr_body.h b/ectrans_amd/csrc/emi_mr_body.h
--- a/ectrans_amd/csrc/emi_mr_body.h
+++ b/ectrans_amd/csrc/emi_mr_body.h
@@ -20,6 +20,10 @@
 #define MR_STAMP_BEGIN() ((void)0)
 #define MR_STAMP(i_) ((void)0)
 #define MR_STAMP_END() ((void)0)
+#endif
+
+#ifndef EMI_MRS_FRONT
+#define EMI_MRS_FRONT 1
 #endif
 
 template <int I, int N, class F>
@@ -145,6 +149,47 @@
   }
 };
 
+template <int R>
+EMI_DEVFN void mr_twiddle(real_t *xr, real_t *xi, real2 w) {
+  if constexpr (sizeof(real_t) == 4 && (R > 8)) {
+    real_t qr[4], qi[4];
+    qr[1] = w.x, qi[1] = w.y;
+    mr_for<1, R>([&](auto rc) {
+      constexpr int r = decltype(rc)::value;
+      if constexpr (r == 2) {
+        qr[2] = w.x * w.x - w.y * w.y, qi[2] = 2 * w.x * w.y;
+      } else if constexpr (r == 3) {
+        qr[3] = qr[2] * w.x - qi[2] * w.y, qi[3] = qr[2] * w.y + qi[2] * w.x;
+      } else if constexpr (r == 4) {
+        qr[0] = qr[2] * qr[2] - qi[2] * qi[2], qi[0] = 2 * qr[2] * qi[2];
+        w = mk2(qr[0], qi[0]);
+      } else if constexpr (r > 4) {
+        const real_t t0 = qr[r & 3] * w.x - qi[r & 3] * w.y;
+        qi[r & 3] = qr[r & 3] * w.y + qi[r & 3] * w.x, qr[r & 3] = t0;
+      }
+      const real_t t1 = xr[r] * qr[r & 3] - xi[r] * qi[r & 3];
+      xi[r] = xr[r] * qi[r & 3] + xi[r] * qr[r & 3], xr[r] = t1;
+    });
+  } else {
+    real_t cr = w.x, ci = w.y;
+    mr_for<1, R>([&](auto rc) {
+      constexpr int r = decltype(rc)::value;
+      if constexpr (r > 1) {
+        const real_t t0 = cr * w.x - ci * w.y;
+        ci = cr * w.y + ci * w.x, cr = t0;
+      }
+      const real_t t1 = xr[r] * cr - xi[r] * ci;
+      xi[r] = xr[r] * ci + xi[r] * cr, xr[r] = t1;
+    });
+  }
+}
+
+EMI_DEVFN real2 mr_fout_pair(real2 za, real2 zb, real2 w, real_t sc) {
+  const real2 s1 = cadd(za, cconj(zb)), d1 = csub(za, cconj(zb));
+  const real2 tt = cmuli(cmul(w, d1));
+  return mk2((s1.x - tt.x) * sc, (s1.y - tt.y) * sc);
+}
+
 EMI_DEVFN unsigned mr_magic(unsigned D) { return D > 1 ? 0xFFFFFFFFu / D + 1u : 0u; }
 EMI_DEVFN unsigned mr_div(unsigned j, unsigned m) { return m ? (unsigned)(((unsigned long long)j * m) >> 32) : j; }
 
@@ -513,3 +558,205 @@
     }
   }
 }
+
+template <int A_, int B_, int C_, int NT_, int FBK_>
+struct MrsPlan {
+  static_assert(FBK_ == 1, "k_fft_*_mrs: one field per workgroup");
+  static constexpr int A = A_, B = B_, C = C_, NT = NT_;
+  static constexpr int sz = A * B * C, n = 2 * sz, BC = B * C, P1 = BC | 1, fs = A * P1;
+  static constexpr int last = C > 1 ? 2 : (B > 1 ? 1 : 0);
+  static constexpr int word = A | (B << 8) | (C << 16) | (FBK_ << 24);
+};
+
+template <class PL, int IP, int IO>
+EMI_DEVFN void mrs_pass(real2 *a, const EmiBuf &b_tw, const EmiBuf &b_row) {
+  constexpr int R = IP == 0 ? PL::A : (IP == 1 ? PL::B : PL::C);
+  constexpr int cnt = PL::sz / R;
+  constexpr int D = IP == 0 ? 1 : (IP == 1 ? PL::C : PL::A);
+  constexpr int SU = IP == 0 ? 1 : (IP == 1 ? PL::P1 : PL::C);
+  constexpr int SV = IP == 0 ? 0 : (IP == 1 ? 1 : PL::P1);
+  constexpr int ES = IP == 0 ? PL::P1 : (IP == 1 ? PL::C : 1);
+  constexpr unsigned SZ2 = sizeof(real2);
+#pragma unroll 1
+  for (unsigned j = (unsigned)EMI_TID; j < (unsigned)cnt; j += (unsigned)PL::NT) {
+    const unsigned u = j / (unsigned)D, v = j - u * (unsigned)D;
+    real2 *p = a + (u * (unsigned)SU + v * (unsigned)SV);
+    real_t xr[R], xi[R];
+    real2 w = mk2(1, 0);
+    if constexpr (IP == 1) w = emi_buf_ld<real2>(b_tw, u * SZ2, 0);
+    if constexpr (IP == 2) w = emi_buf_ld<real2>(b_tw, j * SZ2, (unsigned)PL::A * SZ2);
+    if constexpr (IO == 1) {
+      mr_for<0, R>([&](auto rc) {
+        constexpr int r = decltype(rc)::value;
+        const real2 z = emi_buf_ld<real2>(b_row, j * SZ2, (unsigned)(cnt * r) * SZ2);
+        xr[r] = z.x, xi[r] = z.y;
+      });
+    } else {
+      mr_for<0, R>([&](auto rc) {
+        constexpr int r = decltype(rc)::value;
+        const real2 z = p[r * ES];
+        xr[r] = z.x, xi[r] = z.y;
+      });
+    }
+    if constexpr (IP != 0) mr_twiddle<R>(xr, xi, w);
+    MrDft<R>::run(xr, xi, [&](auto kc, real_t re, real_t im) {
+      constexpr int k = decltype(kc)::value;
+      if constexpr (IO == 2)
+        emi_buf_st<real2>(b_row, j * SZ2, (unsigned)(cnt * k) * SZ2, mk2(re, -im));
+      else
+        p[k * ES] = mk2(re, im);
+    });
+  }
+}
+
+EMI_DEVFN EmiBuf mrs_row_buf(const GridFld &gf, unsigned gpoff, int nproma, int n) {
+  const unsigned blk0 = gpoff / (unsigned)nproma, rem0 = gpoff - blk0 * (unsigned)nproma;
+  return emi_buf(emi_uniform_ptr(mr_row(gf, (long long)blk0, rem0, nproma)), (unsigned)n * (unsigned)sizeof(real_t));
+}
+
+template <class PL>
+EMI_DEVFN void mrs_dir_plan(real2 *a, const FftRowDev &rw_, const FftTabDev &T, int adj, const GridFld *flds, int f0, real_t *FB, int ldf, int nproma) {
+  constexpr unsigned SZ2 = sizeof(real2);
+  constexpr int NT = PL::NT;
+  const int nmen = rw_.nmen;
+  const GridFld gf = flds[f0];
+  const EmiBuf b_tw = emi_buf_all((const real2 *)T.ptw + rw_.ptw_off0);
+  const EmiBuf b_rtw = emi_buf((const real2 *)T.rtw + rw_.rtw_off, (unsigned)(PL::sz + 1) * SZ2);
+  const EmiBuf b_row = mrs_row_buf(gf, (unsigned)rw_.gpoff, nproma, PL::n);
+  const unsigned rowb = (unsigned)ldf * (unsigned)sizeof(real_t);
+  const EmiBuf b_fb = emi_buf(emi_uniform_ptr(FB + (unsigned long long)(unsigned)rw_.fb0 * (unsigned)ldf + 2 * f0), (unsigned)nmen * rowb + SZ2);
+  const real_t sc = (real_t)0.5 * (adj ? (real_t)1.0 : (real_t)(rw_.rw / (double)PL::n)) * fft_dir_mode_scale(gf.mode, (real_t)rw_.racthe);
+  mrs_pass<PL, 0, 1>(a, b_tw, b_row);
+  constexpr bool FRONT = EMI_MRS_FRONT && PL::B <= 16 && PL::C <= 16;
+  real2 w4[4];
+  if constexpr (FRONT) {
+#pragma unroll
+    for (int e = 0; e < 4; e++) w4[e] = emi_buf_ld<real2>(b_rtw, (unsigned)(EMI_TID + e * NT) * SZ2, 0);
+  }
+  auto sync = [&]() {
+    if constexpr (FRONT)
+      EMI_LDS_SYNC();
+    else
+      EMI_SYNC();
+  };
+  if constexpr (PL::B > 1) {
+    sync();
+    mrs_pass<PL, 1, 0>(a, b_tw, b_row);
+  }
+  if constexpr (PL::C > 1) {
+    sync();
+    mrs_pass<PL, 2, 0>(a, b_tw, b_row);
+  }
+  sync();
+  auto pos = [&](unsigned k) {
+    const unsigned q1 = k / (unsigned)PL::A, k3 = k / (unsigned)(PL::A * PL::B);
+    return (k - q1 * (unsigned)PL::A) * (unsigned)PL::P1 + (q1 - k3 * (unsigned)PL::B) * (unsigned)PL::C + k3;
+  };
+  for (unsigned k0 = (unsigned)EMI_TID; k0 <= (unsigned)nmen; k0 += 4u * (unsigned)NT) {
+    real2 za[4], zb[4];
+    if (!FRONT || k0 >= 4u * (unsigned)NT) {
+#pragma unroll
+      for (int e = 0; e < 4; e++) w4[e] = emi_buf_ld<real2>(b_rtw, (k0 + (unsigned)(e * NT)) * SZ2, 0);
+    }
+#pragma unroll
+    for (int e = 0; e < 4; e++) {
+      const unsigned k = k0 + (unsigned)(e * NT);
+      if (k <= (unsigned)nmen) za[e] = a[pos(k)], zb[e] = a[pos(k == 0 ? 0u : (unsigned)PL::sz - k)];
+    }
+#pragma unroll
+    for (int e = 0; e < 4; e++) {
+      const unsigned k = k0 + (unsigned)(e * NT);
+      if (k <= (unsigned)nmen) emi_buf_st<real2>(b_fb, k * rowb, 0, mr_fout_pair(za[e], zb[e], w4[e], sc));
+    }
+  }
+}
+
+template <class PL>
+EMI_DEVFN void mrs_inv_plan(real2 *a, const FftRowDev &rw_, const FftTabDev &T, int adj, const GridFld *flds, int f0, const real_t *FB, int ldf, int nproma) {
+  constexpr unsigned SZ2 = sizeof(real2);
+  constexpr int NT = PL::NT, sz = PL::sz, npair = sz / 2 + 1;
+  constexpr unsigned pad = PL::BC > 1 ? (unsigned)(PL::P1 - PL::BC) : 0u;
+  const int nmen = rw_.nmen;
+  const GridFld gf = flds[f0];
+  const EmiBuf b_tw = emi_buf_all((const real2 *)T.ptw + rw_.ptw_off0);
+  const EmiBuf b_rtw = emi_buf((const real2 *)T.rtw + rw_.rtw_off, (unsigned)(sz + 1) * SZ2);
+  const EmiBuf b_row = mrs_row_buf(gf, (unsigned)rw_.gpoff, nproma, PL::n);
+  const unsigned rowb = (unsigned)ldf * (unsigned)sizeof(real_t);
+  const EmiBuf b_fb = emi_buf(emi_uniform_ptr(FB + (unsigned long long)(unsigned)rw_.fb0 * (unsigned)ldf + 2 * gf.src), (unsigned)nmen * rowb + SZ2);
+  real_t fa, fb;
+  fin_factors(gf.mode, (real_t)rw_.racthe, fa, fb);
+  const real_t fsc = adj ? (real_t)(rw_.rw / (double)PL::n) : (real_t)1.0;
+#pragma unroll 1
+  for (unsigned g0 = (unsigned)EMI_TID; g0 < (unsigned)npair; g0 += 4u * (unsigned)NT) {
+    real2 xa[4], xb[4], w4[4];
+#pragma unroll
+    for (int e = 0; e < 4; e++) {
+      const unsigned k = g0 + (unsigned)(e * NT), k2 = (unsigned)sz - k;
+      xa[e] = emi_buf_ld<real2>(b_fb, k * rowb, 0);
+      xb[e] = emi_buf_ld<real2>(b_fb, k2 * rowb, 0);
+      w4[e] = emi_buf_ld<real2>(b_rtw, k * SZ2, 0);
+    }
+#pragma unroll
+    for (int e = 0; e < 4; e++) {
+      const unsigned k = g0 + (unsigned)(e * NT), k2 = (unsigned)sz - k;
+      if (k < (unsigned)npair) {
+        real2 zk, zk2;
+        fin_pair(xa[e], xb[e], k, k2, fa, fb, fsc, cconj(w4[e]), mk2((real_t)1.0, (real_t)0.0), mk2((real_t)1.0, (real_t)0.0), zk, zk2);
+        a[k + (pad ? k / (unsigned)PL::BC * pad : 0u)] = cconj(zk);
+        if (k2 != k && k2 < (unsigned)sz) a[k2 + (pad ? k2 / (unsigned)PL::BC * pad : 0u)] = cconj(zk2);
+      }
+    }
+  }
+  EMI_SYNC();
+  if constexpr (PL::last == 0)
+    mrs_pass<PL, 0, 2>(a, b_tw, b_row);
+  else
+    mrs_pass<PL, 0, 0>(a, b_tw, b_row);
+  if constexpr (PL::B > 1) {
+    EMI_SYNC();
+    if constexpr (PL::last == 1)
+      mrs_pass<PL, 1, 2>(a, b_tw, b_row);
+    else
+      mrs_pass<PL, 1, 0>(a, b_tw, b_row);
+  }
+  if constexpr (PL::C > 1) {
+    EMI_SYNC();
+    mrs_pass<PL, 2, 2>(a, b_tw, b_row);
+  }
+}
+
+EMI_KERNEL_MRS(4) void k_fft_dir_mrs(FftTabDev T, FftLaunchDev Lc, const GridFld *flds, real_t *FB, int ldf, int nproma) {
+  EMI_LDS_DECL;
+  real2 *a = (real2 *)EMI_LDS_PTR;
+  const int bid = (int)xcd_swizzle(EMI_BID, Lc.nblocks, 8);
+  const int li = bid / Lc.nchunk;
+  const FftRowDev rw_ = Lc.rows[li];
+  const int f0 = bid - li * Lc.nchunk;
+  switch (rw_.mr_abc) {
+#define EMI_MRS_CASE(id_, n_, a_, b_, c_, nt_, fbk_)                                                       \
+  case MrsPlan<a_, b_, c_, nt_, fbk_>::word:                                                               \
+    mrs_dir_plan<MrsPlan<a_, b_, c_, nt_, fbk_>>(a, rw_, T, Lc.adj, flds, f0, FB, ldf, nproma);            \
+    break;
+    EMI_MRS_PLAN_LIST(EMI_MRS_CASE)
+#undef EMI_MRS_CASE
+    default: break;
+  }
+}
+
+EMI_KERNEL_MRS(4) void k_fft_inv_mrs(FftTabDev T, FftLaunchDev Lc, const GridFld *flds, const real_t *FB, int ldf, int nproma) {
+  EMI_LDS_DECL;
+  real2 *a = (real2 *)EMI_LDS_PTR;
+  const int bid = (int)xcd_swizzle(EMI_BID, Lc.nblocks, 8);
+  const int li = bid / Lc.nchunk;
+  const FftRowDev rw_ = Lc.rows[li];
+  const int f0 = bid - li * Lc.nchunk;
+  switch (rw_.mr_abc) {
+#define EMI_MRS_CASE(id_, n_, a_, b_, c_, nt_, fbk_)                                                       \
+  case MrsPlan<a_, b_, c_, nt_, fbk_>::word:                                                               \
+    mrs_inv_plan<MrsPlan<a_, b_, c_, nt_, fbk_>>(a, rw_, T, Lc.adj, flds, f0, FB, ldf, nproma);            \
+    break;
+    EMI_MRS_PLAN_LIST(EMI_MRS_CASE)
+#undef EMI_MRS_CASE
+    default: break;
+  }
+}
diff --git a/ectrans_amd/csrc/emi_mrs_list.h b/ectrans_amd/csrc/emi_mrs_list.h
--- /dev/null
+++ b/ectrans_amd/csrc/emi_mrs_list.h
@@ -0,0 +1,35 @@
+#pragma once
+#define EMI_MRS_PLAN_LIST_F64(X) \
+  X(1, 5120, 10, 16, 16, 256, 1) \
+  X(2, 5100, 10, 15, 17, 256, 1) \
+  X(3, 5096, 13, 14, 14, 256, 1) \
+  X(4, 5040, 12, 14, 15, 256, 1) \
+  X(5, 5016, 11, 12, 19, 256, 1) \
+  X(6, 4992, 12, 13, 16, 256, 1) \
+  X(7, 4940, 10, 13, 19, 256, 1) \
+  X(8, 4928, 11, 14, 16, 256, 1) \
+  X(9, 4896, 12, 12, 17, 256, 1) \
+  X(10, 4864, 8, 16, 19, 256, 1) \
+  X(11, 4800, 10, 15, 16, 256, 1) \
+  X(12, 4788, 9, 14, 19, 256, 1) \
+  X(13, 4760, 10, 14, 17, 256, 1) \
+  X(14, 4732, 13, 13, 14, 256, 1) \
+  X(15, 4704, 12, 14, 14, 256, 1) \
+  X(16, 4680, 12, 13, 15, 256, 1) \
+  X(17, 4624, 8, 17, 17, 256, 1) \
+  X(18, 4620, 11, 14, 15, 256, 1) \
+  X(19, 4608, 12, 12, 16, 256, 1) \
+  X(20, 4576, 11, 13, 16, 256, 1) \
+  X(21, 4560, 10, 12, 19, 256, 1) \
+  X(22, 4500, 10, 15, 15, 256, 1) \
+  X(23, 4488, 11, 12, 17, 256, 1) \
+  X(24, 4480, 10, 14, 16, 256, 1) \
+  X(25, 4420, 10, 13, 17, 256, 1) \
+  X(26, 4368, 12, 13, 14, 256, 1) \
+  X(27, 4352, 8, 16, 17, 256, 1) \
+  X(28, 4332, 6, 19, 19, 256, 1) \
+  X(29, 4320, 12, 12, 15, 256, 1) \
+  X(30, 4312, 11, 14, 14, 256, 1) \
+  X(31, 4284, 9, 14, 17, 256, 1) \
+  X(32, 4256, 7, 16, 19, 256, 1)
+#define EMI_MRS_PLAN_LIST_F32(X)
diff --git a/ectrans_amd/csrc/emi_rt.h b/ectrans_amd/csrc/emi_rt.h
--- a/ectrans_amd/csrc/emi_rt.h
+++ b/ectrans_amd/csrc/emi_rt.h
@@ -13,6 +13,7 @@
 #define EMI_KERNEL_LB(T) __global__ __launch_bounds__(T)
 #define EMI_KERNEL_FFT(W) __global__ __attribute__((amdgpu_flat_work_group_size(64, 1024), amdgpu_waves_per_eu(W, W)))
 #define EMI_KERNEL_MR(W) __global__ __attribute__((amdgpu_flat_work_group_size(64, 256), amdgpu_waves_per_eu(W, W)))
+#define EMI_KERNEL_MRS(W) EMI_KERNEL_MR(W)
 #define EMI_KERNEL_LB2(T, W) __global__ __attribute__((amdgpu_flat_work_group_size(T, T), amdgpu_waves_per_eu(W, W)))
 #define EMI_KERNEL_LAM(W) __global__ __attribute__((amdgpu_flat_work_group_size(64, 512), amdgpu_waves_per_eu(W, W)))
 #define EMI_DEVFN __device__ __forceinline__
@@ -112,6 +113,7 @@
 #define EMI_KERNEL_LB2(T, W)
 #define EMI_KERNEL_LAM(W)
 #define EMI_KERNEL_MR(W)
+#define EMI_KERNEL_MRS(W)
 #define EMI_DEVFN inline
 struct EmuCtx {
   int tid, bid, nthreads;
diff --git a/include/ectrans_mi.h b/include/ectrans_mi.h
--- a/include/ectrans_mi.h
+++ b/include/ectrans_mi.h
@@ -179,6 +179,7 @@
 int emi_last_phase_launches(int *l3);
 int emi_last_exchange(double *ms, int *calls, double *bytes_sent);
 int emi_last_fft_launches(long long *kernels);
+int emi_last_fft_mrs_launches(long long *kernels);
 int emi_set_profile(int on);
 int emi_roctx_active(void);
 int emi_set_max_batch(int max_fields);
```

New measurement: 3.031 (median of 6 runs). Within noise of the previous version (+0.7%).
